# PolyChord/PolyChordLite

Hardware: AMD Instinct MI355X
Metric: likelihood evals/sec, 20D Gaussian nlive=2000 (higher is better)
Workload: dtype f64; 1 GPU; configs[1]: 20-D Gaussian, nlive=2000, num_repeats=40, one full run per step; batch_chains=1000, parallelism=repeat-sharded x1, mode=one run at a time per GPU; R runs in step: roofline.in_step

## Files before the change

### polychordlite_amd/csrc/pc_engine.hip

```cpp
#include "pc_state.h"
#include "pc_resume.h"
#include "pc_prior_table.h"
#include "pc_launch.h"
#include <cstdio>
#include <cstdlib>
#include <cstring>
#include <cstdarg>
#include <cmath>
#include <vector>
#include <memory>
#include <string>
#include <chrono>
#include <algorithm>
#include <map>
#include <unordered_map>
#include <atomic>
#include <mutex>
#include <thread>
#include <functional>
#include <exception>
#include <ucontext.h>
#include <array>
#include <sys/mman.h>
#include <unistd.h>
// ... 521 lines not shown
            case CK_CLUSG: { int nbm = 0, nmx = 0; for (size_t x = i; x < j; ++x) { nbm = std::max(nbm, ord[x]->ia[1]); nmx = std::max(nmx, ord[x]->ia[2]); } rc = pc_launch_knn_cluster_sub_many(d, cnt, nbm, nmx, q); } break;
            case CK_CLUS1: { int ndm = 0, nmx = 0, sub = 0; for (size_t x = i; x < j; ++x) { ndm = std::max(ndm, ord[x]->ia[1]); nmx = std::max(nmx, ord[x]->ia[2]); sub |= ord[x]->ia[3] > 0; } rc = pc_launch_knn_cluster_batch_many(&f.S, d, cnt, ndm, nmx, sub, q); } break;
            case CK_SORT: rc = pc_launch_sort_live_many(&f.S, d, cnt, q); break;
            case CK_CONSUME: rc = pc_launch_consume_par_many(&f.S, d, cnt, q); break;
            case CK_FINAL: rc = pc_launch_final_par_many(d, cnt, q); break;
            case CK_APPLY: rc = pc_launch_apply_many(&f.S, d, cnt, 0u, (int)f.a[0], q); break;
            case CK_UPDATE: { int nbm = 0; for (size_t x = i; x < j; ++x) nbm = std::max(nbm, ord[x]->ia[2]); rc = pc_launch_update_fused_many(&f.S, d, cnt, nbm, (int)f.a[0], (int)f.a[1], q); } break;
            }
            if (rc == 0) n_fused += cnt;
            else for (size_t x = i; x < j; ++x) { single(*ord[x], q); n_single++; }
            if (k == CK_BASES_NEXT && st2) {
                HIPCHK(hipEventRecord(ev_next, st2)); next_pending = true;
                if (!seq_open) { seq_launched++; seq_open = true; }
                if (!ev_seq[seq_launched & 3]) ev_seq[seq_launched & 3] = hpool().get_sync_event();
                HIPCHK(hipEventRecord(ev_seq[seq_launched & 3], st2));
            }
            i = j;
        }
        HIPCHK(hipEventRecord(ev[slot], st)); ev_used[slot] = true;
        if (used_st2 && ev2[slot]) { HIPCHK(hipEventRecord(ev2[slot], st2)); ev2_used[slot] = true; }
        pend.clear();
        seq_open = false;
        run_post();
    }
    void destroy()
    {
        for (int k = 0; k < 4; ++k) if (ev_seq[k]) { hpool().put_sync_event(ev_seq[k]); ev_seq[k] = nullptr; }
        for (int k = 0; k < RING; ++k) {
            if (ev_used[k]) (void)hipEventSynchronize(ev[k]);
            if (ev2_used[k]) (void)hipEventSynchronize(ev2[k]);
            if (ev[k]) hpool().put_sync_event(ev[k]);
            if (ev2[k]) hpool().put_sync_event(ev2[k]);
            ev2[k] = nullptr; ev2_used[k] = false;
            if (h_stage[k]) hfree(h_stage[k]);
            if (d_recs[k]) dfree(d_recs[k]);
            ev[k] = nullptr; h_stage[k] = nullptr; d_recs[k] = nullptr; ev_used[k] = false;
        }
        cap = 0;
    }
};

static std::atomic<long long> g_dbg_compact_ns{0}, g_dbg_nursery_ns{0}, g_dbg_capacity_ns{0}, g_dbg_endb_ns{0}, g_dbg_destroy_ns{0}, g_dbg_evwait_ns{0}, g_dbg_d1{0}, g_dbg_d2{0};
struct Engine {
    Cohort *co = nullptr;
    Fiber *fib = nullptr;
    pchip_settings cfg{};
    std::atomic<int> stop{0};
    polychord_batch_fn batch_fn = nullptr; void *batch_user = nullptr;
    polychord_loglike_fn cb_like = nullptr; polychord_prior_fn cb_prior = nullptr;
    bool callback_mode = false;
    void *d_cs = nullptr; double *d_x0s = nullptr, *d_prop = nullptr;
    int *d_decks = nullptr;
    double *hp_prop = nullptr, *hp_ans = nullptr, *d_ans = nullptr; int *hp_need = nullptr;
    long long cb_evals = 0; long cb_ticks = 0;
    std::vector<int> cb_idx; std::vector<double> cb_c, cb_t, cb_p, cb_l;
    polychord_dumper_fn dumper = nullptr;
    pchip_update_fn on_update = nullptr; void *hook_user = nullptr;
    long ndiscarded = 0;
    bool resume_static = true; unsigned resume_batch0 = 0;
    bool nph_stale = false;
    std::vector<double> hm_dead, hm_logw; int hm_ndead = 0;
    std::vector<unsigned> hm_cuid;
    std::vector<double> pp_rows, pp_logpost; std::vector<unsigned> pp_cuid; std::vector<unsigned long long> pp_uid; int nd_last_update = 0;
    std::vector<unsigned> split_child, split_parent; std::vector<double> split_logfrac;
    std::vector<double> h_lo, h_hi;
    PcState S{};
    hipStream_t st = nullptr;
    hipStream_t st_copy = nullptr;
    bool st_copy_shared = false;
    hipStream_t st_side = nullptr;
    hipEvent_t ev_main = nullptr;
    static constexpr int RAW_RING = 4;
    struct RawSlot { hipEvent_t ready = nullptr, consumed = nullptr; unsigned batch = 0; int B = 0; bool valid = false, waited = false, used = false; int co_seq = 0; };
    RawSlot ring[RAW_RING];
    int raw_depth = 2;
    double *h_dead = nullptr; size_t h_dead_cap = 0, h_dead_copied = 0;
    PcCtl *h_ctl = nullptr;
    PcCtl *h_note = nullptr;
    unsigned note_seq = 0;
    hipEvent_t ev_apply = nullptr;
    double *raw_buf[RAW_RING] = {nullptr, nullptr, nullptr, nullptr};
    double *ph2 = nullptr, *phL2 = nullptr; unsigned *phC2 = nullptr; unsigned long long *phU2 = nullptr;
    unsigned char *keep = nullptr; int *blk = nullptr, *d_total = nullptr;
    double *psum = nullptr, *mean = nullptr, *pcov = nullptr; int *pcnt = nullptr, *count = nullptr;
    size_t cov_chunks_cap = 0;
    double *upd_part = nullptr, *upd_shift = nullptr; size_t upd_part_cap = 0;
    PcPriorTable ptab; bool have_ptab = false;
    double *d_lo = nullptr, *d_hi = nullptr, *d_invcovT = nullptr, *d_mean = nullptr, *d_src = nullptr;
    double *d_dynL = nullptr; int *d_dynN = nullptr; double *d_logn = nullptr;
    double *c_Sm = nullptr; int *c_pts = nullptr, *c_gidx = nullptr, *c_knn = nullptr, *c_lab = nullptr, *c_out = nullptr, *c_cnt = nullptr;
    unsigned *c_olduid = nullptr; int c_cap = 0;
    long nsplits = 0; int ncluster_peak = 1;
    bool src_terms = false;
    long path[PCHIP_PATH_COUNT] = {};
    Timing tm;
    KTimer kt;
    int B = 0, dev = 0;
    bool fast_ok = false;
    bool cb_auto_batch = false; int B_small = 1; double cb_eval_seconds = -1.0;
    long long nlike_g[PC_MAX_GRADE] = {0};
    std::vector<int> h_nlike_g;

    void alloc_phantom_side(int Pcap)
    {
        ph2 = dalloc<double>((size_t)Pcap * S.nT); phL2 = dalloc<double>(Pcap); phC2 = dalloc<unsigned>(Pcap);
        phU2 = dalloc<unsigned long long>(Pcap); keep = dalloc<unsigned char>(Pcap); blk = dalloc<int>((Pcap + 255) / 256 + 1);
    }

    std::vector<void *> setup_staged;
    void upload(void *dst, const void *src, size_t bytes)
    {
        void *h = halloc<char>(bytes);
        setup_staged.push_back(h);
        std::memcpy(h, src, bytes);
        HIPCHK(hipMemcpyAsync(dst, h, bytes, hipMemcpyHostToDevice, st));
    }
    void setup(const pchip_settings &c, const pchip_like &like, const pchip_prior &prior)
    {
        cfg = c;
        { std::lock_guard<std::mutex> g(g_cb_mutex); batch_fn = g_batch_fn; batch_user = g_batch_user; }
        int ndev = 0;
        if (hipGetDeviceCount(&ndev) != hipSuccess || ndev == 0) {
            engine_fail(PC_RC_DEVICE, "no HIP device available -- this engine has no CPU path");
        }
        dev = c.device >= 0 ? c.device % ndev : 0;
        HIPCHK(hipSetDevice(dev));
        st = co ? co->st : hpool().get_stream();
        st_copy = (co && co->stc[0]) ? co->stc[(co->n_stc++) & 1] : (co ? hpool().get_stream() : stream_beside({st}));
        st_copy_shared = co && co->stc[0];
        kt.on = c.profile != 0 && !co; kt.st = st;
        kt.mask = (c.profile == 1) ? 0xFFFFFFFFu : (((unsigned)c.profile >> 1) & 0x7Fu);
        kt.stride = std::max(1u, ((unsigned)c.profile >> 8) & 0xFFu);
        const int D = c.nDims, nDer = c.nDerived;
        S.D = D; S.nDer = nDer; S.nT = 2 * D + nDer + 2; S.nr = c.num_repeats; S.N = c.nlive;
        S.ngrade = 1; S.g_off[0] = 0; S.g_nr[0] = c.num_repeats;
        for (int g = 1; g < PC_MAX_GRADE; ++g) { S.g_off[g] = 0; S.g_nr[g] = 0; }
        if (c.nGrade > 1 && c.grade_dims && c.grade_repeats) {
            if (c.nGrade > PC_MAX_GRADE) engine_fail(PC_RC_SETTINGS, "at most %d parameter grades", PC_MAX_GRADE);
            S.ngrade = c.nGrade;
            int off = 0, tot = 0;
            for (int g = 0; g < c.nGrade; ++g) {
                if (c.grade_dims[g] < 1 || c.grade_repeats[g] < 1) engine_fail(PC_RC_SETTINGS, "every grade needs at least one parameter and one repeat");
                S.g_off[g] = off; off += c.grade_dims[g]; S.g_nr[g] = c.grade_repeats[g]; tot += c.grade_repeats[g];
            }
            if (off != D) engine_fail(PC_RC_SETTINGS, "grade_dims must sum to nDims");
            S.nr = tot; cfg.num_repeats = tot;
        }
        S.nb_total = 0; S.n_dev = 0;
        for (int g = 0, col = 0; g < PC_MAX_GRADE; ++g) {
            const int Dg = D - S.g_off[g];
            S.g_nb[g] = g < S.ngrade ? (S.g_nr[g] + Dg - 1) / Dg : 0;
            S.g_col0[g] = col; S.g_e0[g] = (int)S.n_dev;
            col += S.g_nr[g]; S.nb_total += S.g_nb[g]; S.n_dev += (unsigned)S.g_nb[g] * Dg * Dg;
        }
        sub_dims.clear();
        if (c.n_sub_cluster < 0 || (c.n_sub_cluster > 0 && !c.sub_cluster_dims)) engine_fail(PC_RC_SETTINGS, "n_sub_cluster = %d without a list of coordinates", c.n_sub_cluster);
        for (int k = 0; k < c.n_sub_cluster; ++k) {
            const int d = c.sub_cluster_dims[k];
            if (d < 0 || d >= D) engine_fail(PC_RC_SETTINGS, "sub-clustering coordinate %d out of range (nDims = %d; the indices are 0-based)", d, D);
            if (std::find(sub_dims.begin(), sub_dims.end(), d) != sub_dims.end()) engine_fail(PC_RC_SETTINGS, "sub-clustering coordinate %d given twice", d);
            sub_dims.push_back(d);
        }
        S.ch_nlike_g = nullptr;
        std::memset(nlike_g, 0, sizeof(nlike_g));
        S.p0 = D; S.d0 = 2 * D; S.b0 = 2 * D + nDer; S.l0 = S.b0 + 1;
        int nmax = c.nlive;
        for (int i = 0; i < c.n_nlives; ++i) nmax = std::max(nmax, c.nlives[i]);
        const int nprior = c.nprior <= 0 ? c.nlive : c.nprior;
        S.Ncap = std::max(nmax, nprior);
        B = c.batch > 0 ? c.batch : std::max(1, std::min(1024, c.nlive / 2));
        if (B > 65535) engine_fail(PC_RC_LIMIT, "batch = %d chains per nursery: at most 65535", B);
        if (c.sequential_rng) B = 1;
        cb_auto_batch = c.batch <= 0 && !c.sequential_rng && (like.kind == PC_LIKE_CALLBACK || (prior.kind != 1 && prior.kind != PCHIP_PRIOR_TABLE));
        if (cb_auto_batch) B_small = std::max(1, std::min(64, c.nlive / 4));
        S.B = B;
        S.maxc = c.do_clustering ? std::max(2, g_cap_clusters.load()) : 4;
        S.maxc_dead = 4096;
        S.Pcap = (int)std::min<long long>(2000000000LL / S.nT, 4LL * S.nr * S.Ncap + 4LL * B * S.nr + 1024);
        if (g_cap_phantoms.load() > 0) S.Pcap = std::max(g_cap_phantoms.load(), B * S.nr + 16);
        S.Dcap = 64 * S.Ncap + 4 * B + 1024;
        S.k0 = (uint32_t)c.seed; S.k1 = 0x504F4C59u;
        S.logzero = c.logzero; S.use_prec = c.precision_criterion > 0;
        S.log_prec = S.use_prec ? std::log(c.precision_criterion) : 0.0;
        S.log_cf = std::log(c.compression_factor);
        S.max_ndead = c.max_ndead; S.nfail = c.nfail <= 0 ? c.nlive : c.nfail;
        S.seed_override = 0; S.ablate = c.ablate; S.seq_mode = c.sequential_rng ? 1 : 0;
        S.epoch_discard = c.epoch_discard ? 1 : 0;
        if (S.seq_mode) { cfg.batch = 1; cfg.force_general = 1; }
        S.n_nlives = c.n_nlives;
        if (c.n_nlives > 0) {
            d_dynL = dalloc<double>(c.n_nlives); d_dynN = dalloc<int>(c.n_nlives);
            upload(d_dynL, c.loglikes, sizeof(double) * c.n_nlives);
            upload(d_dynN, c.nlives, sizeof(int) * c.n_nlives);
        }
        S.dyn_loglikes = d_dynL; S.dyn_nlives = d_dynN;
        S.like.kind = like.kind; S.like.mu = like.mu; S.like.sigma = like.sigma; S.like.logdetcov = like.logdetcov;
        S.like.norm = -(double)D * (std::log(like.sigma > 0 ? like.sigma : 1.0) + PC_LOG_TWO_PI / 2.0);
        S.like.inv_sigma = like.sigma > 0 ? 1.0 / like.sigma : 1.0;
        S.like.log_vn = 0.5 * D * std::log(3.14159265358979323846) - std::lgamma(1.0 + D / 2.0);
        S.like.invcov = nullptr; S.like.mean = nullptr;
        S.src_id = 0; S.src_pad = 0; S.src_data = nullptr; S.src_ndata = 0;
        if (like.kind == PC_LIKE_SOURCE) {
            const double *h = nullptr; long long n = 0;
            if (pc_rtc_source_data(like.source, &h, &n)) engine_fail(PC_RC_SETTINGS, "device source handle %d does not exist", like.source);
            if (nDer > PC_SRC_MAX_DERIVED) engine_fail(PC_RC_SETTINGS, "a device source likelihood writes at most %d derived parameters, not %d", PC_SRC_MAX_DERIVED, nDer);
            if (prior.kind != 1 && prior.kind != PCHIP_PRIOR_TABLE) engine_fail(PC_RC_SETTINGS, "a device source likelihood needs a device prior (the uniform box), not a host-callback prior");
            S.src_id = like.source;
            src_terms = pc_rtc_source_terms(like.source) > 0;
            if (n > 0) { d_src = dalloc<double>((size_t)n); upload(d_src, h, sizeof(double) * (size_t)n); S.src_data = d_src; S.src_ndata = n; }
        }
        if (like.kind == PC_LIKE_CORR_GAUSSIAN) {
            std::vector<double> T((size_t)D * D);
            for (int a = 0; a < D; ++a) for (int b = 0; b < D; ++b) T[(size_t)b * D + a] = like.invcov[(size_t)a * D + b];
            d_invcovT = dalloc<double>((size_t)D * D); d_mean = dalloc<double>(D);
            upload(d_invcovT, T.data(), sizeof(double) * D * D);
            upload(d_mean, like.mean, sizeof(double) * D);
            S.like.invcov = d_invcovT; S.like.mean = d_mean;
        }
        have_ptab = false;
        int prior_kind = prior.kind;
        std::vector<double> box_lo, box_hi;
        const double *p_lo = prior.lo, *p_hi = prior.hi;
        if (prior.kind == PCHIP_PRIOR_TABLE) {
            const std::string err = pc_prior_table_build(D, prior.table, prior.hyper, ptab);
            if (!err.empty()) { pc_abi_set_last_error(err.c_str()); engine_fail(PC_RC_SETTINGS, "%s", err.c_str()); }
            have_ptab = true;
            if (ptab.is_box && like.kind != PC_LIKE_CALLBACK) {
                box_lo.resize(D); box_hi.resize(D);
                for (int i = 0; i < D; ++i) { box_lo[i] = ptab.e[i].par[0]; box_hi[i] = ptab.e[i].par[1]; }
                prior_kind = 1; p_lo = box_lo.data(); p_hi = box_hi.data();
            }
        } else if (prior.kind != 0 && prior.kind != 1) engine_fail(PC_RC_SETTINGS, "prior.kind = %d: 0 (callback), 1 (uniform box) or 2 (table)", prior.kind);
        callback_mode = (like.kind == PC_LIKE_CALLBACK) || (prior_kind != 1 && prior_kind != PCHIP_PRIOR_TABLE);
        if (callback_mode) {
            cb_like = like.fn; cb_prior = prior.kind == PCHIP_PRIOR_TABLE ? nullptr : prior.fn;
            if (!cb_like) engine_fail(PC_RC_SETTINGS, "callback mode needs a loglikelihood function pointer");
        }
        S.prior.kind = callback_mode ? (prior_kind == PCHIP_PRIOR_TABLE ? 0 : prior_kind) : prior_kind; S.prior.lo = nullptr; S.prior.hi = nullptr;
        if (prior_kind == 1 && p_lo && p_hi) {
            d_lo = dalloc<double>(D); d_hi = dalloc<double>(D);
            upload(d_lo, p_lo, sizeof(double) * D);
            upload(d_hi, p_hi, sizeof(double) * D);
            S.prior.lo = d_lo; S.prior.hi = d_hi;
        }
        if (S.prior.kind == PCHIP_PRIOR_TABLE) {
            const std::vector<double> tp = ptab.dev_par(); const std::vector<int> ti = ptab.dev_int();
            d_lo = dalloc<double>(tp.size()); d_hi = dalloc<double>((ti.size() + 1) / 2);
            upload(d_lo, tp.data(), sizeof(double) * tp.size());
            upload(d_hi, ti.data(), sizeof(int) * ti.size());
            S.prior.lo = d_lo; S.prior.hi = d_hi; S.src_pad = (int)ptab.mask;
        }
        const int Ncap = S.Ncap, maxc = S.maxc, nT = S.nT, nr = S.nr;
        S.live = dalloc<double>((size_t)Ncap * nT); S.live_logL = dalloc<double>(Ncap);
        S.live_cluster = dalloc<int>(Ncap); S.live_pos = dalloc<int>(Ncap); S.live_entry = dalloc<double>(Ncap);
        S.cl_list = dalloc<int>((size_t)maxc * Ncap); S.cl_n = dalloc<int>(maxc);
        S.logZp = dalloc<double>(maxc); S.logXp = dalloc<double>(maxc); S.logZXp = dalloc<double>(maxc);
        S.logZp2 = dalloc<double>(maxc); S.logZpXp = dalloc<double>(maxc); S.logLp = dalloc<double>(maxc);
        S.XpXq = dalloc<double>(2 * (size_t)maxc * maxc); S.imin_slot = dalloc<int>(maxc);
        S.lse_ref = dalloc<double>(maxc); S.lse_sum = dalloc<double>(maxc); S.death_thr = dalloc<double>(maxc);
        S.cl_uid = dalloc<unsigned>(maxc);
        S.chol = dalloc<double>((size_t)maxc * D * D); S.cov = dalloc<double>((size_t)maxc * D * D);
        S.logZp_dead = dalloc<double>(S.maxc_dead); S.logZp2_dead = dalloc<double>(S.maxc_dead); S.cl_uid_dead = dalloc<unsigned>(S.maxc_dead);
        S.phantom = dalloc<double>((size_t)S.Pcap * nT); S.ph_logL = dalloc<double>(S.Pcap);
        S.ph_cuid = dalloc<unsigned>(S.Pcap); S.ph_uid = dalloc<unsigned long long>(S.Pcap);
        alloc_phantom_side(S.Pcap);
        S.dead = dalloc<double>((size_t)S.Dcap * nT); S.dead_logw = dalloc<double>(S.Dcap);
        S.dead_postX = dalloc<double>(S.Dcap); S.dead_postZ = dalloc<double>(S.Dcap); S.dead_cuid = dalloc<unsigned>(S.Dcap);
        S.dead_entry = dalloc<double>(S.Dcap);
        S.babies = dalloc<double>((size_t)B * nr * nT); S.baby_logL = dalloc<double>((size_t)B * nr); S.baby_logL_T = dalloc<double>((size_t)B * nr);
        S.ch_cluster = dalloc<int>(B); S.ch_epoch = dalloc<int>(B); S.ch_nlike = dalloc<int>(B); S.ch_seed_slot = dalloc<int>(B);
        S.ch_contour = dalloc<double>(B);
        if (S.ngrade > 1) { S.ch_nlike_g = dalloc<int>((size_t)B * PC_MAX_GRADE); h_nlike_g.assign((size_t)B * PC_MAX_GRADE, 0); }
        {
            std::vector<double> ln((size_t)Ncap + 4);
            ln[0] = -PC_HUGE;
            for (int k = 1; k < Ncap + 4; ++k) ln[k] = std::log((double)k);
            d_logn = dalloc<double>(ln.size());
            upload(d_logn, ln.data(), sizeof(double) * ln.size());
            S.logn = d_logn;
        }
        S.nn_list = nullptr; S.nn_slot_owner = nullptr; S.nn_chain_slot = nullptr; S.nn_pts = nullptr; S.nn_code = nullptr; S.nn_valid = 0;
        if (c.do_clustering) {
            S.nn_list = dalloc<int>((size_t)B * nr * PC_NN_K); S.nn_slot_owner = dalloc<int>(Ncap); S.nn_chain_slot = dalloc<int>(B);
            S.nn_pts = dalloc<double>((size_t)(Ncap + B) * D); S.nn_code = dalloc<int>((size_t)2 * Ncap + B + 64);
            if (!sub_dims.empty()) { c_subdims = dalloc<int>(sub_dims.size()); upload(c_subdims, sub_dims.data(), sizeof(int) * sub_dims.size()); }
        }
        S.nhat = dalloc<double>((size_t)B * nr * D); S.nhat_w = dalloc<double>((size_t)B * nr);
        static const bool ms_off = std::getenv("PC_MS_PRE_OFF") != nullptr;
        const bool ms_pre = S.like.kind == PC_LIKE_CORR_GAUSSIAN && D > 64 && D <= 128 && S.ngrade <= 1 && !S.seq_mode && !(S.ablate & 1) && !ms_off && S.prior.kind != PCHIP_PRIOR_TABLE;
        S.nhat_Ms = ms_pre ? dalloc<double>((size_t)B * nr * D) : nullptr;
        S.ch_My = ms_pre ? dalloc<double>((size_t)B * D) : nullptr;
        static const bool split_off = std::getenv("PC_NHATS_SPLIT_OFF") != nullptr;
        const bool split_q = D > 64 && D <= 128 && S.ngrade <= 1 && !S.seq_mode && !split_off && !callback_mode;
        const bool split_m = D > 24 && D <= 64 && S.ngrade <= 1 && !S.seq_mode && !split_off && !callback_mode;
        const size_t raw_n = split_q ? (size_t)B * S.nb_total * 32 * 512 : split_m ? (size_t)B * S.nb_total * (D <= 32 ? 1024 : 4096) : (size_t)B * S.nb_total * D * D + (size_t)B * 33 + 8;
        S.nhat_raw = ((D <= 24 && !S.seq_mode && !split_off) || split_q || split_m) ? dalloc<double>(raw_n)
                   : (D > 128 ? dalloc<double>((size_t)B * S.nb_total * D * 256) : nullptr);
        static const int depth_env = std::getenv("PC_RAW_DEPTH") ? std::max(2, std::min(RAW_RING, std::atoi(std::getenv("PC_RAW_DEPTH")))) : 3;
        raw_depth = split_q ? RAW_RING : depth_env;
        raw_buf[0] = S.nhat_raw;
        for (int r = 1; r < raw_depth; ++r) raw_buf[r] = ((D <= 24 || split_q || split_m) && S.nhat_raw) ? dalloc<double>(raw_n) : nullptr;
        S.plan = dalloc<PcPlan>(B); S.slot_src = dalloc<int>(Ncap); S.slot_step = dalloc<int>(Ncap); S.slot_dead = dalloc<int>(Ncap); HIPCHK(hipMemsetAsync(S.slot_dead, 0xFF, sizeof(int) * Ncap, st)); S.defer_update = 0; S.sort_slot = dalloc<int>(Ncap + 64); S.sort_key = dalloc<unsigned long long>(Ncap + 64);
        S.ctl = dalloc<PcCtl>(1);
        d_total = dalloc<int>(1);
        if (callback_mode) {
            d_cs = (void *)dalloc<char>(pc_chain_state_size() * B); d_x0s = dalloc<double>((size_t)B * D); d_prop = dalloc<double>((size_t)B * D);
            const size_t nans = (size_t)B * (1 + D + std::max(1, nDer));
            d_ans = dalloc<double>(nans);
            d_decks = dalloc<int>((size_t)B * nr);
            hp_prop = halloc<double>((size_t)B * D); hp_ans = halloc<double>(nans); hp_need = halloc<int>(B);
            std::memset(hp_ans, 0, sizeof(double) * nans); std::memset(hp_need, 0, sizeof(int) * B);
            HIPCHK(hipMemset(d_cs, 0, pc_chain_state_size() * B));
        }
        h_ctl = halloc<PcCtl>(1);
        h_note = halloc<PcCtl>(1);
        std::memset(h_note, 0, sizeof(PcCtl)); note_seq = 0;
        { void *dp = nullptr; HIPCHK(hipHostGetDevicePointer(&dp, h_note, 0)); S.ctl_host = (PcCtl *)dp; }
        S.notify_seq = 0;
        pc_launch_init_state(&S, c.logzero, st);
        PcCtl c0{};
        c0.status = PC_ST_RUNNING; c0.ncluster = 1; c0.logZ = c.logzero; c0.logZ2 = c.logzero;
        c0.logX_last_update = 0.0; c0.next_cluster_uid = 1; c0.live_logZ = c.logzero;
        *h_ctl = c0;
    }

    void grade_counts(long *o)
    {
        for (int g = 0; g < PC_MAX_GRADE; ++g) o[g] = 0;
        if (S.ngrade <= 1) { o[0] = (long)h_ctl->nlike; return; }
        long rest = 0;
        for (int g = 1; g < S.ngrade; ++g) { o[g] = (long)nlike_g[g]; rest += o[g]; }
        o[0] = (long)h_ctl->nlike - rest;
    }

    void tally_grades()
    {
        if (S.ngrade <= 1) return;
        for (int w = h_ctl->seg_lo; w <= h_ctl->seg_hi; ++w)
            for (int g = 0; g < PC_MAX_GRADE; ++g) nlike_g[g] += h_nlike_g[(size_t)w * PC_MAX_GRADE + g];
    }

    void sync_point()
    {
        if (fib) {
            fib->yield();
            if (fib->cancel) {
                for (const Fetch &f : fetching) hfree(f.h);
                fetching.clear(); own_fetches.clear();
                for (void *h : staged_up) hfree(h);
                staged_up.clear();
                throw FiberCancelled{};
            }
            return;
        }
        if (co) co->flush();
        for (int spins = 0; spins < 200000; ++spins) { const hipError_t q = hipStreamQuery(st); if (q != hipErrorNotReady) { HIPCHK(q); break; } __builtin_ia32_pause(); }
        HIPCHK(hipStreamSynchronize(st));
    }
    void direct_op() { if (co) co->flush(); }
    struct Fetch { void *h; void *dst; size_t bytes; };
    std::vector<Fetch> fetching;
    void fetch_raw(void *dst, const void *src, size_t bytes)
    {
        if (!bytes) return;
        void *h = halloc<char>(bytes);
        fetching.push_back({h, dst, bytes});
        hipStream_t q = st;
        if (co && batch_copies()) co->post_copies.push_back({(uintptr_t)h, (uintptr_t)src, (uintptr_t)bytes});
        else if (co) co->post.push_back([h, src, bytes, q] { HIPCHK(hipMemcpyAsync(h, src, bytes, hipMemcpyDeviceToHost, q)); });
        else if (batch_copies()) own_fetches.push_back({(uintptr_t)h, (uintptr_t)src, (uintptr_t)bytes});
        else HIPCHK(hipMemcpyAsync(h, src, bytes, hipMemcpyDeviceToHost, st));
    }
    template <class T> void fetch(std::vector<T> &v, const T *p, size_t n) { v.resize(n); fetch_raw(v.data(), p, sizeof(T) * n); }
    std::vector<std::array<uintptr_t, 3>> own_fetches;
    void fetch_wait()
    {
        if (!own_fetches.empty()) { std::vector<std::array<uintptr_t, 3>> c; c.swap(own_fetches); pc_copy_many(c, st); }
        sync_point();
        for (const Fetch &f : fetching) { std::memcpy(f.dst, f.h, f.bytes); hfree(f.h); }
        fetching.clear();
        for (void *h : staged_up) hfree(h);
        staged_up.clear();
    }
    std::vector<void *> staged_up;
    void send_raw(void *dst, const void *src, size_t bytes)
    {
        if (!bytes) return;
        direct_op();
        void *h = halloc<char>(bytes);
        staged_up.push_back(h);
        std::memcpy(h, src, bytes);
        if (co && batch_copies()) co->pre_copies.push_back({(uintptr_t)dst, (uintptr_t)h, (uintptr_t)bytes});
        else HIPCHK(hipMemcpyAsync(dst, h, bytes, hipMemcpyHostToDevice, st));
    }

    void send_pre(void *dst, const void *src, size_t bytes)
    {
        if (!bytes) return;
        if (!co) { send_raw(dst, src, bytes); return; }
        void *h = halloc<char>(bytes);
        staged_up.push_back(h);
        std::memcpy(h, src, bytes);
        hipStream_t q = st;
        if (batch_copies()) co->pre_copies.push_back({(uintptr_t)dst, (uintptr_t)h, (uintptr_t)bytes});
        else co->pre.push_back([dst, h, bytes, q] { HIPCHK(hipMemcpyAsync(dst, h, bytes, hipMemcpyHostToDevice, q)); });
    }
    static bool batch_copies() { static const bool off = std::getenv("PC_COPY_BATCH_OFF") != nullptr; return !off; }

    void read_ctl()
    {
        fetch_raw(h_ctl_in(), S.ctl, sizeof(PcCtl));
        fetch_wait();
        *h_ctl = ctl_in;
        HIPCHK(hipGetLastError());
        nph_stale = false;
        kt.collect();
    }
    PcCtl ctl_in;
    PcCtl *h_ctl_in() { return &ctl_in; }

    void launch_stamp() { S.notify_seq = ++note_seq; }
    unsigned long ready_spins = 0;
    bool round_ready()
    {
        static const bool off = std::getenv("PC_NOTIFY_OFF") != nullptr;
        if (off || !S.ctl_host) { read_ctl(); return true; }
        const volatile unsigned long long *w = (const volatile unsigned long long *)h_note;
        unsigned long long got[PC_NOTE_WORDS];
        bool all = true;
        for (int i = 0; i < PC_NOTE_WORDS; ++i) { got[i] = w[i]; all = all && (unsigned)(got[i] >> 32) == note_seq; }
        if (!all) {
            if ((++ready_spins & 0x3FFFu) == 0x3FFFu) {
                const hipError_t q = hipStreamQuery(st);
                if (q == hipSuccess) {
                    bool ok = true;
                    for (int i = 0; i < PC_NOTE_WORDS; ++i) ok = ok && (unsigned)(w[i] >> 32) == note_seq;
                    if (!ok) engine_fail(PC_RC_DEVICE, "a contraction kernel finished without reporting (launch failure?)");
                } else if (q != hipErrorNotReady) engine_fail(PC_RC_DEVICE, "HIP error %s while waiting for a round", hipGetErrorString(q));
                if (ready_spins > (1ul << 22)) std::this_thread::yield();
            }
            return false;
        }
        PcCtl &c = *h_ctl;
        const int hi_before = c.i_nursery > 0 ? c.i_nursery - 1 : B - 1;
        c.status = (int)(got[0] & 0xFF); c.error = (int)((got[0] >> 8) & 0xFF); c.cluster_deleted = (int)((got[0] >> 16) & 1);
        c.upd_pending = (int)((got[0] >> 17) & 1); c.upd_marks = (int)((got[0] >> 18) & 0x3FFF);
        c.i_nursery = (int)((unsigned)got[1] & 0xFFFFu); c.ndead = (int)(unsigned)got[2]; c.nphantom = (int)(unsigned)got[3];
        c.ncluster = (int)(got[4] & 0xFFFF);
        {
            int cand = (c.ncluster_dead & ~0xFFFF) | (int)((got[4] >> 16) & 0xFFFF);
            if (cand < c.ncluster_dead) cand += 0x10000;
            c.ncluster_dead = cand;
        }
        c.seg_hi = hi_before; c.seg_lo = c.i_nursery;
        nph_stale = false;
        return true;
    }

    void grow_dead(int nd)
    {
        if (co) co->flush();
        HIPCHK(hipStreamSynchronize(st_copy));
        auto grow = [&](auto *&p, size_t per) {
            using T = std::remove_reference_t<decltype(*p)>;
            T *q = dalloc<T>((size_t)nd * per);
            HIPCHK(hipMemcpyAsync(q, p, sizeof(T) * (size_t)h_ctl->ndead * per, hipMemcpyDeviceToDevice, st));
            HIPCHK(hipStreamSynchronize(st));
            dfree(p); p = q;
        };
        grow(S.dead, S.nT); grow(S.dead_logw, 1); grow(S.dead_postX, 1); grow(S.dead_postZ, 1); grow(S.dead_cuid, 1); grow(S.dead_entry, 1);
        S.Dcap = nd;
        if (h_dead && (size_t)nd > h_dead_cap) { hfree(h_dead); h_dead_cap = (size_t)nd; h_dead = halloc<double>(h_dead_cap * S.nT); h_dead_copied = 0; }
    }

    void grow_phantoms(long long need)
    {
        if (co) co->flush();
        const long long hard = 1LL << 30;
        if (need > hard) engine_fail(PC_RC_LIMIT, "more than %lld phantom points (%lld needed)", hard, need);
        long long np = std::max<long long>(need, 2LL * S.Pcap);
        np = std::min(np, hard);
        if (g_inject_fault.load() == 3) { g_inject_fault = 0; engine_fail(PC_RC_MEMORY, "out of device memory growing the phantom array to %lld rows (injected)", np); }
        const size_t used = (size_t)std::min<long long>(h_ctl->nphantom, S.Pcap);
        HIPCHK(hipStreamSynchronize(st));
        auto grow = [&](auto *&p, size_t per) {
            using T = std::remove_reference_t<decltype(*p)>;
            T *q = dalloc<T>((size_t)np * per);
            if (used) HIPCHK(hipMemcpyAsync(q, p, sizeof(T) * used * per, hipMemcpyDeviceToDevice, st));
            HIPCHK(hipStreamSynchronize(st));
            dfree(p); p = q;
        };
        grow(S.phantom, S.nT); grow(S.ph_logL, 1); grow(S.ph_cuid, 1); grow(S.ph_uid, 1);
        dfree(ph2); dfree(phL2); dfree(phC2); dfree(phU2); dfree(keep); dfree(blk);
        alloc_phantom_side((int)np);
        S.Pcap = (int)np;
    }

    long long pool_cursor = 0;
    double *babies_own = nullptr;
    bool compact_wanted() const { return S.pool && h_ctl->status == PC_ST_RUNNING && h_ctl->i_nursery == 0 && pool_cursor + (long long)B * S.nr > S.Pcap; }
    void compact_record() { co->rec(CK_COMPACT, S, {keep, blk, d_total, ph2, phL2, phC2, phU2}, {}, {0, (int)pool_cursor, ((int)pool_cursor + 255) / 256}); }
    void compact_finish(int total)
    {
        std::swap(S.phantom, ph2); std::swap(S.ph_logL, phL2); std::swap(S.ph_cuid, phC2); std::swap(S.ph_uid, phU2);
        pool_cursor = total; h_ctl->nphantom = total; nph_stale = false;
        if (pool_cursor + (long long)B * S.nr > S.Pcap / 2) grow_phantoms(std::max<long long>(2LL * S.Pcap, 2 * (pool_cursor + (long long)B * S.nr)));
        tm.compactions++;
    }
    void pool_compact()
    {
        const auto dbg_t0 = std::chrono::steady_clock::now();
        struct DbgT { std::chrono::steady_clock::time_point t0; ~DbgT() { g_dbg_compact_ns += std::chrono::duration_cast<std::chrono::nanoseconds>(std::chrono::steady_clock::now() - t0).count(); } } dbg_t{dbg_t0};
        if (co) co->flush();
        hipEvent_t e0 = kt.begin(KT_CLEAN);
        pc_launch_clean(&S, (int)pool_cursor, keep, blk, d_total, ph2, phL2, phC2, phU2, nullptr, st);
        kt.end(KT_CLEAN, e0);
        int total = 0;
        HIPCHK(hipMemcpyAsync(&total, d_total, sizeof(int), hipMemcpyDeviceToHost, st));
        HIPCHK(hipStreamSynchronize(st));
        kt.collect();
        compact_finish(total);
    }
    void ensure_capacity()
    {
        if ((long long)h_ctl->ndead + B + S.Ncap + 16 > S.Dcap) grow_dead(S.Dcap * 2);
        if (S.pool) { if (h_ctl->ncluster_dead + h_ctl->ncluster + 8 > S.maxc_dead) grow_dead_clusters(2 * S.maxc_dead); return; }
        if (nph_stale && (long long)h_ctl->nphantom + (long long)B * S.nr > S.Pcap) read_ctl();
        if ((long long)h_ctl->nphantom + (long long)B * S.nr > S.Pcap) grow_phantoms((long long)h_ctl->nphantom + (long long)B * S.nr);
        if (h_ctl->ncluster_dead + h_ctl->ncluster + 8 > S.maxc_dead) grow_dead_clusters(2 * S.maxc_dead);
    }

    void grow_dead_clusters(int nd)
    {
        if (co) co->flush();
        HIPCHK(hipStreamSynchronize(st));
        const size_t used = (size_t)std::min(h_ctl->ncluster_dead, S.maxc_dead);
        auto grow = [&](auto *&p) {
            using T = std::remove_reference_t<decltype(*p)>;
            T *q = dalloc<T>((size_t)nd);
            if (used) HIPCHK(hipMemcpy(q, p, sizeof(T) * used, hipMemcpyDeviceToDevice));
            dfree(p); p = q;
        };
        grow(S.logZp_dead); grow(S.logZp2_dead); grow(S.cl_uid_dead);
        S.maxc_dead = nd;
    }

    void grow_clusters(int need)
    {
        const int mo = S.maxc, mn = std::max(need, 2 * mo), Ncap = S.Ncap, DD = S.D * S.D;
        if (mn > 16384) engine_fail(PC_RC_LIMIT, "more than 16384 clusters");
        if (co) co->flush();
        HIPCHK(hipStreamSynchronize(st));
        auto grow_d = [&](double *&p, double fill) {
            std::vector<double> v = dl(p, (size_t)mo); v.resize(mn, fill);
            dfree(p); p = dalloc<double>(mn); ul(p, v);
        };
        grow_d(S.logZp, cfg.logzero); grow_d(S.logZXp, cfg.logzero); grow_d(S.logZp2, cfg.logzero); grow_d(S.logZpXp, cfg.logzero);
        grow_d(S.logLp, cfg.logzero); grow_d(S.logXp, 0.0); grow_d(S.lse_ref, 0.0); grow_d(S.lse_sum, 0.0); grow_d(S.death_thr, -PC_HUGE);
        { std::vector<int> v = dl(S.cl_n, (size_t)mo); v.resize(mn, 0); dfree(S.cl_n); S.cl_n = dalloc<int>(mn); ul(S.cl_n, v); }
        { std::vector<int> v = dl(S.imin_slot, (size_t)mo); v.resize(mn, 0); dfree(S.imin_slot); S.imin_slot = dalloc<int>(mn); ul(S.imin_slot, v); }
        { std::vector<unsigned> v = dl(S.cl_uid, (size_t)mo); v.resize(mn, 0u); dfree(S.cl_uid); S.cl_uid = dalloc<unsigned>(mn); ul(S.cl_uid, v); }
        {
            std::vector<double> o = dl(S.XpXq, (size_t)mo * mo), v((size_t)mn * mn, 0.0);
            for (int a = 0; a < mo; ++a) std::copy(o.begin() + (size_t)a * mo, o.begin() + (size_t)(a + 1) * mo, v.begin() + (size_t)a * mn);
            dfree(S.XpXq); S.XpXq = dalloc<double>(2 * (size_t)mn * mn); ul(S.XpXq, v);
        }
        {
            int *q = dalloc<int>((size_t)mn * Ncap);
            HIPCHK(hipMemcpy(q, S.cl_list, sizeof(int) * (size_t)mo * Ncap, hipMemcpyDeviceToDevice));
            dfree(S.cl_list); S.cl_list = q;
        }
        auto grow_mat = [&](double *&p) {
            double *q = dalloc<double>((size_t)mn * DD);
            HIPCHK(hipMemcpy(q, p, sizeof(double) * (size_t)mo * DD, hipMemcpyDeviceToDevice));
            std::vector<double> id((size_t)(mn - mo) * DD, 0.0);
            for (int c = 0; c < mn - mo; ++c) for (int a = 0; a < S.D; ++a) id[(size_t)c * DD + (size_t)a * S.D + a] = 1.0;
            HIPCHK(hipMemcpy(q + (size_t)mo * DD, id.data(), sizeof(double) * id.size(), hipMemcpyHostToDevice));
            dfree(p); p = q;
        };
        grow_mat(S.chol); grow_mat(S.cov);
        if (c_cnt) { dfree(c_cnt); dfree(c_olduid); c_cnt = dalloc<int>(mn); c_olduid = dalloc<unsigned>(mn); }
        dfree(psum); dfree(pcnt); dfree(pcov); dfree(mean); dfree(count); cov_chunks_cap = 0;
        S.maxc = mn;
    }

    void call_dumper(int stage = 0)
    {
        if (!(dumper && stage != 2) && !on_update) return;
        const int nT = S.nT, D = S.D, nDer = S.nDer, npars = D + nDer + 2, nd = h_ctl->ndead;
        HIPCHK(hipStreamSynchronize(st));
        if (nd > hm_ndead) {
            std::vector<double> rows((size_t)(nd - hm_ndead) * nT), lw(nd - hm_ndead);
            hm_cuid.resize(nd);
            HIPCHK(hipMemcpy(hm_cuid.data() + hm_ndead, S.dead_cuid + hm_ndead, sizeof(unsigned) * (nd - hm_ndead), hipMemcpyDeviceToHost));
            HIPCHK(hipMemcpy(rows.data(), S.dead + (size_t)hm_ndead * nT, sizeof(double) * rows.size(), hipMemcpyDeviceToHost));
            HIPCHK(hipMemcpy(lw.data(), S.dead_logw + hm_ndead, sizeof(double) * lw.size(), hipMemcpyDeviceToHost));
            hm_dead.resize((size_t)nd * npars); hm_logw.resize(nd);
            for (int i = hm_ndead; i < nd; ++i) {
                const double *r = rows.data() + (size_t)(i - hm_ndead) * nT;
                double *o = hm_dead.data() + (size_t)i * npars;
                std::memcpy(o, r + S.p0, sizeof(double) * (D + nDer)); o[D + nDer] = r[S.b0]; o[D + nDer + 1] = r[S.l0];
                hm_logw[i] = lw[i - hm_ndead] + r[S.l0];
            }
            hm_ndead = nd;
        }
        std::vector<double> lwn(hm_logw.begin(), hm_logw.begin() + nd);
        double m = -PC_HUGE;
// ... 1781 lines not shown
```

### polychordlite_amd/csrc/pc_launch.h

```cpp
#pragma once
#include "pc_state.h"
#include "../../include/polychord_hip.h"
#include <cstddef>

static inline int pc_slice_phi_lds(const PcState *S)
{
    const size_t sh0 = sizeof(double) * ((size_t)S->D + S->nr) + 16, tb = sizeof(double) * (size_t)S->nr * (S->D + 1);
    return (S->nDer > 0 && sh0 + tb <= 48 * 1024) ? 1 : 0;
}

extern "C" {

void pc_abi_set_last_error(const char *msg);
void pc_launch_slice_tick(const PcState *S, unsigned batch, int nchains, void *cs, double *x0s, int *decks, double *prop, const double *ev_logL,
                          const double *ev_theta, const double *ev_phi, int first, double *prop_host, int *need_host, hipStream_t st);
size_t pc_chain_state_size(void);
int pc_launch_killoff_cl(const PcState *S, int nc, hipStream_t st);
int pc_consume_cl_fits(const PcState *S, int nc);
int pc_consume_clp_fits(const PcState *S, int nc);
int pc_launch_consume_cl_many(const PcState *S, const PcManyRec *dR, int R, int wide, hipStream_t st);
int pc_launch_consume_cl(const PcState *S, int nc, hipStream_t st);
int pc_launch_knn_cluster_sub(const int *d_desc, int nb, int mmax, const double *Sm, const int *pool, int *knn, int *labels, int *out, hipStream_t st);
int pc_launch_knn_cluster_sub_many(const PcManyRec *dR, int R, int nb_max, int mmax, hipStream_t st);
void pc_launch_remap_chains(const PcState *S, const int *map, int nold, int n, hipStream_t st);
void pc_launch_shift_mats(const PcState *S, int p, int nc, hipStream_t st);
void pc_launch_similarity(const PcState *S, const int *pts, int n, double *Sm, const int *dims, int nd, hipStream_t st);
int pc_launch_knn_cluster(const double *Sm, int nroot, const int *gidx, int m, int *knn, int *labels, int *out, hipStream_t st);
int pc_launch_knn_cluster_batch(const PcState *S, const int *h_desc, const int *d_desc, int nd, double *Sm, int *knn, int *labels, int *out, const int *dims, int ndims, hipStream_t st);
int pc_launch_knn_cluster_batch_dev(const PcState *S, const int *d_desc, int nd, int nmax, double *Sm, int *knn, int *labels, int *out, const int *dims, int ndims, hipStream_t st);
int pc_launch_knn_cluster_batch_many(const PcState *S, const PcManyRec *dR, int R, int nd_max, int nmax, int any_sub, hipStream_t st);
void pc_launch_rebuild(const PcState *S, int nc, hipStream_t st);
void pc_launch_ph_rehome(const PcState *S, int nph, int nc, const unsigned *old_uids, int nold_uids, int *counts, hipStream_t st);
void pc_launch_nn_lists(const PcState *S, int nleft, int use_rank, hipStream_t st);
int pc_launch_nn_lists_many(const PcState *S, const PcManyRec *dR, int R, int nleft_max, int use_rank, hipStream_t st);
int pc_launch_consume(const PcState *S, int final_mode, int wide, hipStream_t st);
void pc_launch_apply(const PcState *S, unsigned batch, int nchains, hipStream_t st);
int pc_launch_apply_many(const PcState *S, const PcManyRec *dR, int R, unsigned batch, int nchains, hipStream_t st);
int pc_launch_clean_many(const PcManyRec *dR, int R, int nblk_max, hipStream_t st);
void pc_launch_install_live(const PcState *S, const double *rows, int n, hipStream_t st);
void pc_launch_clean(const PcState *S, int nph, unsigned char *keep, int *blk, int *d_total, double *ph2, double *phL2, unsigned *phC2, unsigned long long *phU2, int *dst_index, hipStream_t st);
void pc_launch_reset_thresholds(const PcState *S, hipStream_t st);
int pc_launch_reset_thresholds_many(const PcState *S, const PcManyRec *dR, int R, hipStream_t st);
int pc_cov_nchunk(const PcState *S, int nph);
int pc_launch_covmats(const PcState *S, int nph, int nc, double *psum, int *pcnt, double *mean, int *count, double *pcov, hipStream_t st);
void pc_launch_scan_blocks(int *blk, int nblk, int *total, int *total2, hipStream_t st);
void pc_launch_chol_only(const PcState *S, const double *ncov, const int *count, hipStream_t st);
void pc_launch_init_state(const PcState *S, double logzero, hipStream_t st);
int pc_post_blocks(void);
void pc_launch_post_moments(const PcState *S, int nd, double *pmax, double *part, hipStream_t st);
void pc_prepare_streams(int dev, int want);
void *pc_cache_dev_alloc(size_t bytes);
void pc_cache_dev_free(void *p);
void *pc_cache_host_alloc(size_t bytes);
void pc_cache_host_free(void *p);
int pc_run_many(const pchip_settings *s, const pchip_like *like, const pchip_prior *prior, int nseeds, const int *seeds, int device, int max_in_flight, pchip_result *results);
int pc_fast_fits(const PcState *S);
int pc_launch_sort_live(const PcState *S, hipStream_t st);
int pc_launch_sort_live_many(const PcState *S, const PcManyRec *dR, int R, hipStream_t st);
int pc_launch_consume_fast(const PcState *S, int final_mode, hipStream_t st);
void pc_launch_ph_prepare(const PcState *S, hipStream_t st);
size_t pc_records_block_bytes(long long cap, int nT);
int pc_pack_lived_device(const double *dead, const double *logw, const double *entry, long long nd, int nT, double logzero, double *block, long long cap, long long *h_count, hipStream_t st);
int pc_par_fits(const PcState *S);
int pc_launch_consume_par(const PcState *S, hipStream_t st);
int pc_launch_consume_par_many(const PcState *S, const PcManyRec *dR, int R, hipStream_t st);
int pc_launch_final_par(const PcState *S, hipStream_t st);
int pc_launch_final_par_many(const PcManyRec *dR, int R, hipStream_t st);
int pc_rtc_launch(const PcState *S, const char *expr, dim3 grid, dim3 block, size_t sh, hipStream_t st, void **args);
const char *pc_rtc_error(void);
int pc_rtc_source_data(int id, const double **data, long long *n);
long pc_rtc_source_terms(int id);
int pc_rtc_wanted(const PcState *S);
int pc_launch_generate_live(const PcState *S, int attempt0, int n, double *rows, double *rows_logL, hipStream_t st);
int pc_nhats_splittable(const PcState *S);
int pc_launch_nhats_part(const PcState *S, unsigned batch, int nchains, int part, hipStream_t st, int packed);
int pc_launch_nhats(const PcState *S, unsigned batch, int nchains, hipStream_t st);
int pc_slice_fusable(const PcState *S);
int pc_launch_slice_fused(const PcState *S, unsigned batch, int nchains, hipStream_t st);
int pc_launch_slice_many(const PcState *S, const PcManyRec *dR, int R, int nchains, int fused, hipStream_t st);
int pc_launch_nhats_many(const PcState *S, const PcManyRec *dR, int R, int nchains, hipStream_t st);
int pc_launch_slice(const PcState *S, unsigned batch, int nchains, hipStream_t st);
int pc_launch_prior_transform(const PcState *S, int n, const double *cubes, double *thetas, hipStream_t st);
int pc_launch_source_eval(const PcState *S, int n, const double *thetas, double *logL, double *phi, hipStream_t st);
int pc_bases_t_ok(const PcState *S);
int pc_launch_bases_t(const PcState *S, unsigned batch, int nchains, hipStream_t st);
int pc_launch_bases_t_many(const PcState *S, const PcManyRec *dR, int R, unsigned batch, int nchains, hipStream_t st);
int pc_slice_t_ok(const PcState *S, int ncluster);
int pc_launch_slice_t(const PcState *S, unsigned batch, int nchains, hipStream_t st);
int pc_launch_slice_t_many(const PcState *S, const PcManyRec *dR, int R, unsigned batch, int nchains, hipStream_t st);
int pc_update_fused_ok(const PcState *S, int nc);
int pc_update_fused_blocks(const PcState *S, int nph);
int pc_update_fused_entries(const PcState *S);
void pc_launch_update_fused(const PcState *S, int nph, unsigned char *keep, int *blk, int *d_total, double *ph2, double *phL2, unsigned *phC2,
                            unsigned long long *phU2, double *part, double *shift, int deferred, hipStream_t st);
int pc_update_fused_grid(const PcState *S, int nph, int deferred);
int pc_launch_update_fused_many(const PcState *S, const PcManyRec *dR, int R, int nblk_max, int G, int deferred, hipStream_t st);

}
```

### polychordlite_amd/csrc/pc_update.hip

```cpp
#include "pc_state.h"
#include "pc_launch.h"
#include <atomic>
#include <cstdio>
#include <cstdlib>

#define UPD_ROWS 256
#define UPD_NT 256

__device__ __forceinline__ void upd_stage_masked(const double *src0, unsigned long long mask, unsigned long long mmask, double *dst,
                                                 double *tile, int TS, const double *sh, int D, int nT, int lane)
{
    const int ne = dst ? nT : D + 1;
    int n = 0;
    while (mask) {
        int idx[16], cnt = 0;
#pragma unroll
        for (int u = 0; u < 16; ++u) {
            idx[u] = 0;
            if (mask) { idx[u] = __ffsll((long long)mask) - 1; mask &= mask - 1; cnt = u + 1; }
        }
        for (int e = lane; e < ne; e += 64) {
            double v[16];
#pragma unroll
            for (int u = 0; u < 16; ++u) if (u < cnt) v[u] = (e < nT) ? src0[(size_t)idx[u] * nT + e] : 0.0;
            if (dst) {
#pragma unroll
                for (int u = 0; u < 16; ++u) if (u < cnt) dst[(size_t)(n + u) * nT + e] = v[u];
            }
            if (e <= D) {
                const double s = e < D ? sh[e] : 0.0;
#pragma unroll
                for (int u = 0; u < 16; ++u)
                    if (u < cnt && ((mmask >> idx[u]) & 1ull))
                        tile[(size_t)__popcll(mmask & ((1ull << idx[u]) - 1ull)) * TS + e] = e < D ? v[u] - s : 1.0;
            }
        }
        n += cnt;
    }
}

__device__ __forceinline__ void upd_flag_body(const PcState &S, int nph, unsigned char *keep, int *blk_count, int def, int nblk)
{
    const int tid = threadIdx.x, lane = tid & 63, wv = tid >> 6;
    const int sb = blockIdx.x * 4 + wv;
    if (sb >= nblk) return;
    const unsigned uid0 = S.cl_uid[0];
    const double thr = def ? S.ctl->upd_thr : S.death_thr[0];
    const bool pool = S.pool;
    const int tmark = (pool && def) ? S.ctl->upd_tmark : 0x7fffffff, nph0u = (pool && def) ? S.ctl->upd_nph0 : 0x7fffffff;
    const int T = (pool && def) ? S.ctl->upd_T : 0, nr = S.nr;
    const int j0 = sb * UPD_ROWS + 4 * lane;
    const bool full = j0 + 3 < nph;
    unsigned cu[4] = {PC_CUID_NONE, PC_CUID_NONE, PC_CUID_NONE, PC_CUID_NONE};
    double ll[4] = {0.0, 0.0, 0.0, 0.0};
    if (full) {
        const uint4 c = *(const uint4 *)(S.ph_cuid + j0);
        const double2 a = *(const double2 *)(S.ph_logL + j0), b2 = *(const double2 *)(S.ph_logL + j0 + 2);
        cu[0] = c.x; cu[1] = c.y; cu[2] = c.z; cu[3] = c.w; ll[0] = a.x; ll[1] = a.y; ll[2] = b2.x; ll[3] = b2.y;
    } else {
        for (int u = 0; u < 4; ++u) if (j0 + u < nph) { cu[u] = S.ph_cuid[j0 + u]; ll[u] = S.ph_logL[j0 + u]; }
    }
    unsigned kb = 0; bool wr = false; int cnt = 0;
#pragma unroll
    for (int u = 0; u < 4; ++u) {
        const int j = j0 + u;
        bool k = false, km = false;
        if (j < nph) {
            k = (cu[u] == uid0) && !(ll[u] < thr);
            if (pool) {
                if (!k && cu[u] == uid0) { cu[u] = PC_CUID_NONE; wr = true; }
                km = k && (j < nph0u || T - 1 - (j - nph0u) / nr < tmark);
            }
            kb |= (unsigned)((k ? 1 : 0) | (km ? 2 : 0)) << (8 * u);
        }
        cnt += __popcll(__ballot(pool ? km : k));
    }
    if (full) {
        *(unsigned *)(keep + j0) = kb;
        if (wr) *(uint4 *)(S.ph_cuid + j0) = make_uint4(cu[0], cu[1], cu[2], cu[3]);
    } else {
        for (int u = 0; u < 4; ++u) if (j0 + u < nph) { keep[j0 + u] = (unsigned char)((kb >> (8 * u)) & 0xFFu); if (wr) S.ph_cuid[j0 + u] = cu[u]; }
    }
    if (lane == 0) blk_count[sb] = cnt;
}
__global__ __launch_bounds__(UPD_NT) void k_upd_flag(PcState S, int nph, unsigned char *keep, int *blk_count, int def, int nblk) { upd_flag_body(S, nph, keep, blk_count, def, nblk); }
__global__ __launch_bounds__(UPD_NT) void k_upd_flag_many(const PcManyRec *R, int def) { const PcManyView r = pc_many_view(R, blockIdx.y); if ((int)blockIdx.x * 4 >= r.ia[2]) return; upd_flag_body(r.S, r.ia[1], (unsigned char *)r.p[0], (int *)r.p[1], def, r.ia[2]); }


__global__ __launch_bounds__(1024) void k_upd_scan(int *cnt, int n, int *total)
{
    __shared__ int wsum[16];
    __shared__ int carry_s;
    const int tid = threadIdx.x, lane = tid & 63, wv = tid >> 6;
    int carry = 0;
    for (int base = 0; base < n; base += 4096) {
        const int i0 = base + 4 * tid;
        int c[4];
#pragma unroll
        for (int u = 0; u < 4; ++u) c[u] = (i0 + u < n) ? cnt[i0 + u] : 0;
        const int s = (c[0] + c[1]) + (c[2] + c[3]);
        int inc = s;
#pragma unroll
        for (int o = 1; o < 64; o <<= 1) { const int t = __shfl_up(inc, o); if (lane >= o) inc += t; }
        if (lane == 63) wsum[wv] = inc;
        __syncthreads();
        int pre = carry;
        for (int x = 0; x < wv; ++x) pre += wsum[x];
        int run = pre + inc - s;
#pragma unroll
        for (int u = 0; u < 4; ++u) { if (i0 + u < n) cnt[i0 + u] = run; run += c[u]; }
        if (tid == 1023) carry_s = pre + inc;
        __syncthreads();
        carry = carry_s;
    }
    if (tid == 0) *total = carry;
}

__global__ __launch_bounds__(UPD_NT) void k_upd_index(int nph, const unsigned char *keep, const int *blk_off, int *idx)
{
    __shared__ int cnt[4];
    const int tid = threadIdx.x, lane = tid & 63, wv = tid >> 6;
    const int j = blockIdx.x * UPD_ROWS + tid;
    const bool km = j < nph && (keep[j] & 2);
    const unsigned long long m = __ballot(km);
    if (lane == 0) cnt[wv] = __popcll(m);
    __syncthreads();
    int off = blk_off[blockIdx.x];
    for (int x = 0; x < wv; ++x) off += cnt[x];
    if (km) idx[off + __popcll(m & ((1ull << lane) - 1ull))] = j;
}

#define UPD_SELF_BLOCKS 4096
#define UPD_IDX_NT 256
#define UPD_IDX_BLOCKS 16
__device__ __forceinline__ void upd_index_self_body(int nph, const unsigned char *keep, const int *blk_count, int nblk, int *idx, int *total)
{
    __shared__ int part[4];
    const int tid = threadIdx.x, lane = tid & 63, wv = tid >> 6;
    const int sb0 = blockIdx.x * UPD_IDX_BLOCKS;
    int s = 0;
    for (int b = tid; b < sb0; b += UPD_IDX_NT) s += blk_count[b];
#pragma unroll
    for (int o = 32; o >= 1; o >>= 1) s += __shfl_xor(s, o);
    if (lane == 0) part[wv] = s;
    __syncthreads();
    int off = (part[0] + part[1]) + (part[2] + part[3]);
    const int sbw = sb0 + 4 * wv;
    for (int x = sb0; x < sbw && x < nblk; ++x) off += blk_count[x];
    const unsigned long long below = (1ull << lane) - 1ull;
    for (int q = 0; q < 4; ++q) {
        const int sb = sbw + q;
        if (sb >= nblk) return;
        const int j0 = sb * UPD_ROWS + 4 * lane;
        unsigned w = 0;
        if (j0 + 3 < nph) w = *(const unsigned *)(keep + j0);
        else for (int u = 0; u < 4; ++u) if (j0 + u < nph) w |= (unsigned)keep[j0 + u] << (8 * u);
        int pos = off, all = 0;
        bool f[4];
#pragma unroll
        for (int u = 0; u < 4; ++u) {
            f[u] = (w >> (8 * u + 1)) & 1u;
            const unsigned long long m = __ballot(f[u]);
            pos += __popcll(m & below); all += __popcll(m);
        }
#pragma unroll
        for (int u = 0; u < 4; ++u) if (f[u]) { idx[pos] = j0 + u; pos++; }
        off += all;
        if (sb == nblk - 1 && lane == 0) *total = off;
    }
}
__global__ __launch_bounds__(UPD_IDX_NT) void k_upd_index_self(int nph, const unsigned char *keep, const int *blk_count, int nblk, int *idx, int *total) { upd_index_self_body(nph, keep, blk_count, nblk, idx, total); }
__global__ __launch_bounds__(UPD_IDX_NT) void k_upd_index_self_many(const PcManyRec *R) { const PcManyView r = pc_many_view(R, blockIdx.y); if ((int)blockIdx.x * 16 >= r.ia[2]) return; upd_index_self_body(r.ia[1], (const unsigned char *)r.p[0], (const int *)r.p[1], r.ia[2], (int *)r.p[5], (int *)r.p[2]); }


__device__ __forceinline__ void upd_stage_idx(const double *base, const int *ridx, int cnt, double *tile, int TS, const double *sh, int D, int nT, int lane)
{
    if (cnt <= 0) return;
    int idx[16];
#pragma unroll
    for (int u = 0; u < 16; ++u) idx[u] = u < cnt ? ridx[u] : 0;
    for (int e0 = lane; e0 <= D; e0 += 128) {
        const int e1 = e0 + 64;
        double v0[16], v1[16];
#pragma unroll
        for (int u = 0; u < 16; ++u) if (u < cnt) { v0[u] = e0 < D ? base[(size_t)idx[u] * nT + e0] : 1.0; v1[u] = e1 < D ? base[(size_t)idx[u] * nT + e1] : 1.0; }
        const double s0 = e0 < D ? sh[e0] : 0.0, s1 = e1 < D ? sh[e1] : 0.0;
#pragma unroll
        for (int u = 0; u < 16; ++u) if (u < cnt) { tile[(size_t)u * TS + e0] = v0[u] - s0; if (e1 <= D) tile[(size_t)u * TS + e1] = v1[u] - s1; }
    }
}

typedef double upd_v4d __attribute__((ext_vector_type(4)));
template <int NT, int W>
__device__ __forceinline__ void updg_accumulate(const double *tile, int TS, int n16, int wv, int li, int lk, upd_v4d (&acc)[(NT <= 2) ? NT * (NT + 1) / 2 : (NT * (NT + 1) / 2 + 3) / 4])
{
    if constexpr (NT <= 2) {
        for (int q0 = 4 * wv; q0 < n16; q0 += 16) {
            const double *row = tile + (size_t)(q0 + lk) * TS + li;
            double x[NT];
#pragma unroll
            for (int t = 0; t < NT; ++t) x[t] = row[16 * t];
            int q = 0;
#pragma unroll
            for (int ti = 0; ti < NT; ++ti)
#pragma unroll
                for (int tj = ti; tj < NT; ++tj, ++q) acc[q] = __builtin_amdgcn_mfma_f64_16x16x4f64(x[ti], x[tj], acc[q], 0, 0, 0);
        }
    } else {
        for (int ks = 0; ks < (n16 >> 2); ++ks) {
            const double *row = tile + (size_t)(4 * ks + lk) * TS + li;
            double x[NT];
#pragma unroll
            for (int t = 0; t < NT; ++t) x[t] = row[16 * t];
            int q = 0;
#pragma unroll
            for (int ti = 0; ti < NT; ++ti)
#pragma unroll
                for (int tj = ti; tj < NT; ++tj, ++q)
                    if ((q & 3) == W) acc[q >> 2] = __builtin_amdgcn_mfma_f64_16x16x4f64(x[ti], x[tj], acc[q >> 2], 0, 0, 0);
        }
    }
}
__device__ __forceinline__ int updg_slot(int D, int ti, int tj, int li, int lk, int r)
{
    const int a = 16 * ti + lk + 4 * r, b = 16 * tj + li, npair = D * (D + 1) / 2;
    if (a > b || b > D) return -1;
    return (b < D) ? a * D - a * (a - 1) / 2 + (b - a) : (a < D ? npair + a : npair + D);
}

template <int NT, bool IDX>
__device__ __forceinline__ void upd_gather_body(const PcState &S, int nph, int nblk, const unsigned char *keep, const int *blk_off,
                                                double *ph2, double *phL2, unsigned *phC2, unsigned long long *phU2,
                                                const int *idx, const int *nidx_p,
                                                const double *shift, double *part, int E, int def, int nlb, int ndb)
{
    extern __shared__ __attribute__((aligned(16))) char smem[];
    constexpr bool KS = NT <= 2;
    constexpr int TS = KS ? 16 * NT + 1 : 16 * NT + ((NT & 1) ? 0 : 16);
    constexpr int CAP = KS ? 128 : 64;
    constexpr int NACC = KS ? NT * (NT + 1) / 2 : (NT * (NT + 1) / 2 + 3) / 4;
    __shared__ unsigned long long m64[4], mm64[4];
    __shared__ long long dix[256];
    const int tmark = def ? S.ctl->upd_tmark : 0x7fffffff, nph0u = def ? S.ctl->upd_nph0 : 0x7fffffff, updT = def ? S.ctl->upd_T : 0;
    const int tid = threadIdx.x, lane = tid & 63, wv = tid >> 6, li = lane & 15, lk = lane >> 4, D = S.D, nT = S.nT;
    constexpr bool pool = IDX;
    double *tile = (double *)smem;
    double *sh = tile + (size_t)CAP * TS;
    for (int d = tid; d < D; d += 256) sh[d] = shift[d];
    for (int e = tid; e < CAP * TS; e += 256) tile[e] = 0.0;
    upd_v4d acc[NACC];
#pragma unroll
    for (int t = 0; t < NACC; ++t) acc[t] = upd_v4d{0.0, 0.0, 0.0, 0.0};
    int nfill = 0;
    auto flush = [&]() __attribute__((always_inline)) {
        __syncthreads();
        const int n16 = (nfill + 15) & ~15;
        for (int e = tid; e < (n16 - nfill) * (D + 1); e += 256) tile[(size_t)(nfill + e / (D + 1)) * TS + e % (D + 1)] = 0.0;
        __syncthreads();
        if (KS || wv == 0) updg_accumulate<NT, 0>(tile, TS, n16, wv, li, lk, acc);
        else if (wv == 1) updg_accumulate<NT, 1>(tile, TS, n16, wv, li, lk, acc);
        else if (wv == 2) updg_accumulate<NT, 2>(tile, TS, n16, wv, li, lk, acc);
        else updg_accumulate<NT, 3>(tile, TS, n16, wv, li, lk, acc);
        __syncthreads();
        nfill = 0;
    };
    auto piece = [&](const double *src, int sub, double *dst) __attribute__((always_inline)) {
        const unsigned long long ms = m64[sub], mms = mm64[sub], below = (1ull << (16 * wv)) - 1ull;
        const int cnt = __popcll(mms);
        if (cnt == 0 && (dst == nullptr || ms == 0ull)) return;
        if (nfill + cnt > CAP) flush();
        upd_stage_masked(src + (size_t)(sub * 64 + 16 * wv) * nT, ((dst ? ms : mms) >> (16 * wv)) & 0xFFFFull, (mms >> (16 * wv)) & 0xFFFFull,
                         dst ? dst + (size_t)__popcll(ms & below) * nT : nullptr, tile + (size_t)(nfill + __popcll(mms & below)) * TS, TS, sh, D, nT, lane);
        nfill += cnt;
    };
    if constexpr (IDX) {
        const int nidx = *nidx_p;
        const int gchunk = (int)gridDim.x - nlb - ndb;
        for (int c = blockIdx.x; (int)blockIdx.x < gchunk && c * 64 < nidx; c += gchunk) {
            const int have = min(64, nidx - c * 64);
            if (nfill + have > CAP) flush();
            upd_stage_idx(S.phantom, idx + c * 64 + 16 * wv, min(16, have - 16 * wv), tile + (size_t)(nfill + 16 * wv) * TS, TS, sh, D, nT, lane);
            nfill += have;
        }
    }
    const int total = nblk + nlb + ndb;
    for (int b = IDX ? ((int)blockIdx.x >= (int)gridDim.x - nlb - ndb ? nblk + (int)blockIdx.x - ((int)gridDim.x - nlb - ndb) : total) : blockIdx.x; b < total; b += gridDim.x) {
        __syncthreads();
        if (b < nblk) {
            const int j = b * 256 + tid;
            const bool k = (j < nph) && keep[j];
            const bool km = k && (j < nph0u || (pool ? updT - 1 - (j - nph0u) / S.nr : (j - nph0u) / S.nr) < tmark);
            const unsigned long long m = __ballot(k), mm = __ballot(km);
            if (lane == 0) { m64[wv] = m; mm64[wv] = mm; }
            __syncthreads();
            int off = 0;
            if (!pool) {
                off = blk_off[b];
                for (int x = 0; x < wv; ++x) off += __popcll(m64[x]);
                if (k) {
                    const int pos = off + __popcll(m & ((1ull << lane) - 1ull));
                    phL2[pos] = S.ph_logL[j]; phC2[pos] = S.ph_cuid[j]; phU2[pos] = S.ph_uid[j];
                }
                off = blk_off[b];
            }
            const double *src = S.phantom + (size_t)b * 256 * nT;
            for (int sub = 0; sub < 4; ++sub) {
                piece(src, sub, pool ? nullptr : ph2 + (size_t)off * nT);
                off += __popcll(m64[sub]);
            }
        } else if (b < nblk + nlb) {
            const int r0 = (b - nblk) * 256, r = r0 + tid;
            const bool k = (r < S.Ncap) && S.live_cluster[r] == 0 && (!def || S.slot_step[r] < tmark);
            const unsigned long long m = __ballot(k);
            if (lane == 0) { m64[wv] = m; mm64[wv] = m; }
            __syncthreads();
            const double *src = S.live + (size_t)r0 * nT;
            for (int sub = 0; sub < 4; ++sub) piece(src, sub, nullptr);
        } else {
            const PcCtl *ctl = S.ctl;
            const int T = ctl->upd_T, ts = ctl->upd_ts;
            const int t = tmark + (b - nblk - nlb) * 256 + tid;
            long long di = -1;
            if (t < ts) {
                const PcPlan *pw = S.plan + (T - 1 - t);
                const int src = pw->dead_src;
                const bool existed = src >= 0 || (T - 1 - (-src - 1)) < tmark;
                if (pw->dead_idx >= 0 && pw->logw > S.logzero && existed) di = pw->dead_idx;
            }
            dix[tid] = di;
            const unsigned long long m = __ballot(di >= 0);
            if (lane == 0) m64[wv] = m;
            __syncthreads();
            for (int sub = 0; sub < 4; ++sub) {
                unsigned long long mb = m64[sub];
                const int cnt = __popcll(mb);
                if (cnt == 0) continue;
                if (nfill + cnt > CAP) flush();
                int row = 0;
                while (mb) {
                    const int bit = __ffsll((long long)mb) - 1; mb &= mb - 1;
                    if ((row & 3) == wv) {
                        const long long d = dix[sub * 64 + bit];
                        for (int e = lane; e <= D; e += 64) tile[(size_t)(nfill + row) * TS + e] = e < D ? S.dead[(size_t)d * nT + e] - sh[e] : 1.0;
                    }
                    row++;
                }
                nfill += cnt;
            }
        }
    }
    flush();
    double *out = part + (size_t)blockIdx.x * E;
    if constexpr (KS) {
        double *wres = tile;
#pragma unroll
        for (int t = 0; t < NACC; ++t)
#pragma unroll
            for (int r = 0; r < 4; ++r) wres[((size_t)wv * NACC + t) * 256 + (lk + 4 * r) * 16 + li] = acc[t][r];
        __syncthreads();
        if (wv == 0) {
            int q = 0;
#pragma unroll
            for (int ti = 0; ti < NT; ++ti)
#pragma unroll
                for (int tj = ti; tj < NT; ++tj, ++q)
#pragma unroll
                    for (int r = 0; r < 4; ++r) {
                        const int p = updg_slot(D, ti, tj, li, lk, r), idx = (lk + 4 * r) * 16 + li;
                        if (p >= 0) out[p] = ((wres[(size_t)(0 * NACC + q) * 256 + idx] + wres[(size_t)(1 * NACC + q) * 256 + idx]) +
                                              (wres[(size_t)(2 * NACC + q) * 256 + idx] + wres[(size_t)(3 * NACC + q) * 256 + idx]));
                    }
        }
    } else {
        int q = 0;
#pragma unroll
        for (int ti = 0; ti < NT; ++ti)
#pragma unroll
            for (int tj = ti; tj < NT; ++tj, ++q)
                if ((q & 3) == wv) {
#pragma unroll
                    for (int r = 0; r < 4; ++r) { const int p = updg_slot(D, ti, tj, li, lk, r); if (p >= 0) out[p] = acc[q >> 2][r]; }
                }
    }
}
template <int NT, bool IDX>
__global__ __launch_bounds__(256) void k_upd_gather(PcState S, int nph, int nblk, const unsigned char *keep, const int *blk_off,
                                                    double *ph2, double *phL2, unsigned *phC2, unsigned long long *phU2,
                                                    const int *idx, const int *nidx_p,
                                                    const double *shift, double *part, int E, int def, int nlb, int ndb)
{ upd_gather_body<NT, IDX>(S, nph, nblk, keep, blk_off, ph2, phL2, phC2, phU2, idx, nidx_p, shift, part, E, def, nlb, ndb); }
template <int NT>
__global__ __launch_bounds__(256) void k_upd_gather_many(const PcManyRec *R, int E, int def, int nlb, int ndb)
{
    const PcManyView r = pc_many_view(R, blockIdx.y);
    upd_gather_body<NT, true>(r.S, r.ia[1], r.ia[2], (const unsigned char *)r.p[0], (const int *)r.p[1], (double *)r.p[3], (double *)r.p[4], (unsigned *)r.p[5],
                              (unsigned long long *)r.p[6], (const int *)r.p[5], (const int *)r.p[2], (const double *)r.p[8], (double *)r.p[7], E, def, nlb, ndb);
}


#define UPD_FOLD 16
__device__ __forceinline__ void upd_fold_body(const double *part, int nb, int E, double *part2)
{
    const int g = blockIdx.x;
    for (int e = threadIdx.x; e < E; e += 256) {
        double t[UPD_FOLD];
#pragma unroll
        for (int u = 0; u < UPD_FOLD; ++u) t[u] = (g * UPD_FOLD + u < nb) ? part[(size_t)(g * UPD_FOLD + u) * E + e] : 0.0;
        double s = 0.0;
#pragma unroll
        for (int u = 0; u < UPD_FOLD; ++u) s += t[u];
        part2[(size_t)g * E + e] = s;
    }
}
__global__ __launch_bounds__(256) void k_upd_fold(const double *part, int nb, int E, double *part2) { upd_fold_body(part, nb, E, part2); }
__global__ __launch_bounds__(256) void k_upd_fold_many(const PcManyRec *R, int nb, int E) { double *part = pc_as_global((double *)R[blockIdx.y].p[7], R); upd_fold_body(part, nb, E, part + (size_t)nb * E); }


__device__ __forceinline__ void upd_final_body(const PcState &S, int nb, const double *part, int E, double *shift, int def)
{
    __shared__ double acc[4][256];
    __shared__ double A[32 * 32], L[32 * 32], mu[32];
    __shared__ int bad;
    const int tid = threadIdx.x, D = S.D, npair = D * (D + 1) / 2, nE = npair + D + 1;
    __shared__ double tot[544];
    for (int e0 = 0; e0 < nE; e0 += 256) {
        const int e = e0 + (tid & 255), h = tid >> 8;
        double s = 0.0;
        if (e < nE) {
            for (int k = h; k < nb; k += 4 * 16) {
                double t[16];
#pragma unroll
                for (int u = 0; u < 16; ++u) t[u] = (k + 4 * u < nb) ? part[(size_t)(k + 4 * u) * E + e] : 0.0;
#pragma unroll
                for (int u = 0; u < 16; ++u) s += t[u];
            }
        }
        acc[h][tid & 255] = s;
        __syncthreads();
        if (tid < 256 && e < nE) tot[e] = (acc[0][tid] + acc[1][tid]) + (acc[2][tid] + acc[3][tid]);
        __syncthreads();
    }
#ifdef UPD_DBG
    const long long f0 = clock64();
#endif
    if (tid == 0) bad = 0;
    const double n = tot[npair + D];
    if (tid < D) mu[tid] = tot[npair + tid] / n;
    __syncthreads();
    for (int p = tid; p < D * D; p += 1024) {
        const int a = p / D, b = p % D, lo = a < b ? a : b, hi = a < b ? b : a;
        const int idx = lo * D - lo * (lo - 1) / 2 + (hi - lo);
        const double c = tot[idx] / n - mu[lo] * mu[hi];
        A[p] = c; L[p] = 0.0;
        S.cov[p] = c;
    }
    __syncthreads();
#ifdef UPD_DBG
    const long long f1 = clock64();
#endif
    if (tid < 64) {
        double a[32];
#pragma unroll
        for (int k = 0; k < 32; ++k) a[k] = (tid < D && k < D) ? A[tid * D + k] : 0.0;
        bool fail = false;
#pragma unroll
        for (int i = 0; i < 32; ++i) {
            if (i < D && !fail) {
                const double aii = readlane_f64(a[i], i);
                if (aii <= 0.0) fail = true;
                else {
                    const double lii = sqrt(aii);
                    const double lji = (tid == i) ? lii : a[i] / lii;
                    if (tid >= i) a[i] = lji;
#pragma unroll
                    for (int k = i + 1; k < 32; ++k)
                        if (k < D) { const double lki = readlane_f64(lji, k); if (tid > i) a[k] -= lji * lki; }
                }
            }
        }
        if (fail) { if (tid == 0) bad = 1; }
        else if (tid < D) {
#pragma unroll
            for (int k = 0; k < 32; ++k) if (k < D) L[tid * D + k] = (k <= tid) ? a[k] : 0.0;
        }
    }
    __syncthreads();
    if (bad) {
        double tr = 0.0;
        for (int k = 0; k < D; ++k) tr += A[k * D + k];
        for (int p = tid; p < D * D; p += 1024) L[p] = (p / D == p % D) ? sqrt(tr) : 0.0;
        __syncthreads();
    }
    for (int p = tid; p < D * D; p += 1024) S.chol[p] = L[p];
    if (tid < D) shift[tid] += mu[tid];
    if (tid == 0) { if (!(def && S.ctl->upd_keep_thr)) S.death_thr[0] = -PC_HUGE; if (def) S.ctl->upd_pending = 0; }
#ifdef UPD_DBG
    if (tid == 0) { const long long f2 = clock64(); S.ctl->gen_cyc[2] += f1 - f0; S.ctl->gen_cyc[3] += f2 - f1; S.ctl->nn_walks += f0; }
#endif
}
__global__ __launch_bounds__(1024) void k_upd_final(PcState S, int nb, const double *part, int E, double *shift, int def) { upd_final_body(S, nb, part, E, shift, def); }
__global__ __launch_bounds__(1024) void k_upd_final_many(const PcManyRec *R, int nb, int E, int def, int G) { const PcManyView r = pc_many_view(R, blockIdx.y); upd_final_body(r.S, nb, (const double *)r.p[7] + (size_t)G * E, E, (double *)r.p[8], def); }


__global__ __launch_bounds__(1024) void k_upd_final_w(PcState S, int nb, const double *part, int E, double *shift, int def, double *ncov, int *count)
{
    extern __shared__ __attribute__((aligned(16))) char smem[];
    double *tot = (double *)smem;
    __shared__ double mu[128];
    const int tid = threadIdx.x, D = S.D, npair = D * (D + 1) / 2, nE = npair + D + 1;
    for (int e = tid; e < nE; e += 1024) {
        double s = 0.0;
        for (int k = 0; k < nb; k += 8) {
            double t[8];
#pragma unroll
            for (int u = 0; u < 8; ++u) t[u] = (k + u < nb) ? part[(size_t)(k + u) * E + e] : 0.0;
#pragma unroll
            for (int u = 0; u < 8; ++u) s += t[u];
        }
        tot[e] = s;
    }
    __syncthreads();
    const double n = tot[npair + D];
    if (tid < D) mu[tid] = tot[npair + tid] / n;
    __syncthreads();
    for (int p = tid; p < D * D; p += 1024) {
        const int a = p / D, b = p % D, lo = a < b ? a : b, hi = a < b ? b : a;
        ncov[p] = tot[lo * D - lo * (lo - 1) / 2 + (hi - lo)] - n * mu[lo] * mu[hi];
    }
    if (tid < D) shift[tid] += mu[tid];
    if (tid == 0) { count[0] = (int)n; if (!(def && S.ctl->upd_keep_thr)) S.death_thr[0] = -PC_HUGE; if (def) S.ctl->upd_pending = 0; }
}

static int upd_grid(const PcState *S, int nph, int deferred)
{
    const int nblk = (nph + UPD_ROWS - 1) / UPD_ROWS, nlb = (S->Ncap + UPD_ROWS - 1) / UPD_ROWS, ndb = deferred ? (S->B + UPD_ROWS - 1) / UPD_ROWS : 0;
    static const int cap_env = std::getenv("PC_UPD_GRID") ? std::atoi(std::getenv("PC_UPD_GRID")) : 0;
    const int cap = cap_env > 0 ? cap_env : (S->D < 32 ? 384 : 512);
    if (S->pool) { const int nch = (nph + 63) / 64; return (nch < cap ? (nch > 0 ? nch : 1) : cap) + nlb + ndb; }
    const int total = nblk + nlb + ndb;
    return total < cap ? total : cap;
}

extern "C" int pc_update_fused_ok(const PcState *S, int nc) { return nc == 1 && S->D <= 128; }
extern "C" int pc_update_fused_blocks(const PcState *S, int nph)
{
    const int G = upd_grid(S, nph, 1), E = pc_update_fused_entries(S);
    return G + (G + UPD_FOLD - 1) / UPD_FOLD + (S->D * S->D + 2 + E - 1) / E;
}
extern "C" int pc_update_fused_entries(const PcState *S) { const int e = S->D * (S->D + 1) / 2 + S->D + 1; return (e + 31) & ~31; }

extern "C" void pc_launch_update_fused(const PcState *S, int nph, unsigned char *keep, int *blk, int *d_total, double *ph2, double *phL2,
                                       unsigned *phC2, unsigned long long *phU2, double *part, double *shift, int deferred, hipStream_t st)
{
    const int D = S->D, nblk = (nph + UPD_ROWS - 1) / UPD_ROWS, nlb = (S->Ncap + UPD_ROWS - 1) / UPD_ROWS, E = pc_update_fused_entries(S);
    const int ndb = deferred ? (S->B + UPD_ROWS - 1) / UPD_ROWS : 0;
    const int NTv = (D + 1 + 15) / 16, TSv = NTv <= 2 ? 16 * NTv + 1 : 16 * NTv + ((NTv & 1) ? 0 : 16), CAPv = NTv <= 2 ? 128 : 64;
    const int G = upd_grid(S, nph, deferred), ng = (G + UPD_FOLD - 1) / UPD_FOLD;
    double *part2 = part + (size_t)G * E;
    size_t shw = sizeof(double) * ((size_t)CAPv * TSv + D);
    if (NTv <= 2 && shw < sizeof(double) * (size_t)(4 * 3 * 256)) shw = sizeof(double) * (size_t)(4 * 3 * 256);
    hipLaunchKernelGGL(k_upd_flag, dim3((nblk + 3) / 4), dim3(UPD_NT), 0, st, *S, nph, keep, blk, deferred, nblk);
    if (!S->pool) pc_launch_scan_blocks(blk, nblk, d_total, &S->ctl->nphantom, st);
    else if (nblk <= UPD_SELF_BLOCKS && !std::getenv("PC_UPD_SCAN_LAUNCH"))
        hipLaunchKernelGGL(k_upd_index_self, dim3((nblk + 15) / 16), dim3(UPD_IDX_NT), 0, st, nph, (const unsigned char *)keep, (const int *)blk, nblk, (int *)phC2, d_total);
    else {
        hipLaunchKernelGGL(k_upd_scan, dim3(1), dim3(1024), 0, st, blk, nblk, d_total);
        hipLaunchKernelGGL(k_upd_index, dim3(nblk), dim3(UPD_NT), 0, st, nph, (const unsigned char *)keep, (const int *)blk, (int *)phC2);
    }
    int devi = 0; (void)hipGetDevice(&devi); devi &= 63;
#define UPDG_LAUNCH(NT) { \
        pc_need_dyn_lds((const void *)k_upd_gather<NT, false>, shw); \
                          pc_need_dyn_lds((const void *)k_upd_gather<NT, true>, shw); \
         \
        if (S->pool) hipLaunchKernelGGL((k_upd_gather<NT, true>), dim3(G), dim3(256), shw, st, *S, nph, nblk, (const unsigned char *)keep, (const int *)blk, \
                           ph2, phL2, phC2, phU2, (const int *)phC2, (const int *)d_total, (const double *)shift, part, E, deferred, nlb, ndb); \
        else hipLaunchKernelGGL((k_upd_gather<NT, false>), dim3(G), dim3(256), shw, st, *S, nph, nblk, (const unsigned char *)keep, (const int *)blk, \
                           ph2, phL2, phC2, phU2, (const int *)nullptr, (const int *)nullptr, (const double *)shift, part, E, deferred, nlb, ndb); }
    switch (NTv) { case 1: UPDG_LAUNCH(1) break; case 2: UPDG_LAUNCH(2) break; case 3: UPDG_LAUNCH(3) break; case 4: UPDG_LAUNCH(4) break;
                   case 5: UPDG_LAUNCH(5) break; case 6: UPDG_LAUNCH(6) break; case 7: UPDG_LAUNCH(7) break; case 8: UPDG_LAUNCH(8) break;
                   default: UPDG_LAUNCH(9) break; }
#undef UPDG_LAUNCH
    hipLaunchKernelGGL(k_upd_fold, dim3(ng), dim3(256), 0, st, (const double *)part, G, E, part2);
    if (D < 32) { hipLaunchKernelGGL(k_upd_final, dim3(1), dim3(1024), 0, st, *S, ng, (const double *)part2, E, shift, deferred); return; }
    double *ncov = part2 + (size_t)ng * E;
    int *count = (int *)(ncov + (size_t)D * D);
    const size_t shf = sizeof(double) * (size_t)(D * (D + 1) / 2 + D + 1);
    pc_need_dyn_lds((const void *)k_upd_final_w, shf);
    hipLaunchKernelGGL(k_upd_final_w, dim3(1), dim3(1024), shf, st, *S, ng, (const double *)part2, E, shift, deferred, ncov, count);
    pc_launch_chol_only(S, ncov, count, st);
}

extern "C" int pc_update_fused_grid(const PcState *S, int nph, int deferred) { return upd_grid(S, nph, deferred); }
extern "C" int pc_launch_update_fused_many(const PcState *S, const PcManyRec *dR, int R, int nblk_max, int G, int deferred, hipStream_t st)
{
    const int D = S->D, nlb = (S->Ncap + UPD_ROWS - 1) / UPD_ROWS, E = pc_update_fused_entries(S);
    if (!S->pool || nblk_max > UPD_SELF_BLOCKS || D >= 32 || nblk_max < 1) return 1;
    const int ndb = deferred ? (S->B + UPD_ROWS - 1) / UPD_ROWS : 0;
    const int NTv = (D + 1 + 15) / 16, TSv = NTv <= 2 ? 16 * NTv + 1 : 16 * NTv + ((NTv & 1) ? 0 : 16), CAPv = NTv <= 2 ? 128 : 64;
    const int ng = (G + UPD_FOLD - 1) / UPD_FOLD;
    size_t shw = sizeof(double) * ((size_t)CAPv * TSv + D);
    if (NTv <= 2 && shw < sizeof(double) * (size_t)(4 * 3 * 256)) shw = sizeof(double) * (size_t)(4 * 3 * 256);
    hipLaunchKernelGGL(k_upd_flag_many, dim3((nblk_max + 3) / 4, R), dim3(UPD_NT), 0, st, dR, deferred);
    hipLaunchKernelGGL(k_upd_index_self_many, dim3((nblk_max + 15) / 16, R), dim3(UPD_IDX_NT), 0, st, dR);
    int devi = 0; (void)hipGetDevice(&devi); devi &= 63;
#define UPDM_LAUNCH(NT) { \
        pc_need_dyn_lds((const void *)k_upd_gather_many<NT>, shw); \
        hipLaunchKernelGGL((k_upd_gather_many<NT>), dim3(G, R), dim3(256), shw, st, dR, E, deferred, nlb, ndb); }
    if (NTv == 1) UPDM_LAUNCH(1) else UPDM_LAUNCH(2)
#undef UPDM_LAUNCH
    hipLaunchKernelGGL(k_upd_fold_many, dim3(ng, R), dim3(256), 0, st, dR, G, E);
    hipLaunchKernelGGL(k_upd_final_many, dim3(1, R), dim3(1024), 0, st, dR, ng, E, deferred, G);
    return 0;
}
```

Before: 1.218 billion likelihood evals/s.

## Chain covariance update kernels with atomic tickets and shrink final kernel

Adds a fused flag+scan kernel and a chained gather kernel that use last-block atomic tickets, so the separate scan, index, fold and final launches of the covariance update can be merged into fewer launches. The gather path now builds index lists on the fly from block offsets, and dead-point staging uses compacted int indices with a shared staging helper. The final Cholesky kernel is templated on dimension bound and launched with 256 instead of 1024 threads. The new chained path only runs when an ablate bit (1<<16) is set, so by default only the reworked dead staging, the smaller final kernel and the write-through stores take effect.

```diff
diff --git a/polychordlite_amd/csrc/pc_engine.hip b/polychordlite_amd/csrc/pc_engine.hip
--- a/polychordlite_amd/csrc/pc_engine.hip
+++ b/polychordlite_amd/csrc/pc_engine.hip
@@ -847,7 +847,7 @@
         for (int r = 1; r < raw_depth; ++r) raw_buf[r] = ((D <= 24 || split_q || split_m) && S.nhat_raw) ? dalloc<double>(raw_n) : nullptr;
         S.plan = dalloc<PcPlan>(B); S.slot_src = dalloc<int>(Ncap); S.slot_step = dalloc<int>(Ncap); S.slot_dead = dalloc<int>(Ncap); HIPCHK(hipMemsetAsync(S.slot_dead, 0xFF, sizeof(int) * Ncap, st)); S.defer_update = 0; S.sort_slot = dalloc<int>(Ncap + 64); S.sort_key = dalloc<unsigned long long>(Ncap + 64);
         S.ctl = dalloc<PcCtl>(1);
-        d_total = dalloc<int>(1);
+        d_total = dalloc<int>(PC_UPD_CTR_INTS); HIPCHK(hipMemsetAsync(d_total, 0, sizeof(int) * PC_UPD_CTR_INTS, st));
         if (callback_mode) {
             d_cs = (void *)dalloc<char>(pc_chain_state_size() * B); d_x0s = dalloc<double>((size_t)B * D); d_prop = dalloc<double>((size_t)B * D);
             const size_t nans = (size_t)B * (1 + D + std::max(1, nDer));
diff --git a/polychordlite_amd/csrc/pc_launch.h b/polychordlite_amd/csrc/pc_launch.h
--- a/polychordlite_amd/csrc/pc_launch.h
+++ b/polychordlite_amd/csrc/pc_launch.h
@@ -91,6 +91,7 @@
 int pc_update_fused_ok(const PcState *S, int nc);
 int pc_update_fused_blocks(const PcState *S, int nph);
 int pc_update_fused_entries(const PcState *S);
+#define PC_UPD_CTR_INTS 2048
 void pc_launch_update_fused(const PcState *S, int nph, unsigned char *keep, int *blk, int *d_total, double *ph2, double *phL2, unsigned *phC2,
                             unsigned long long *phU2, double *part, double *shift, int deferred, hipStream_t st);
 int pc_update_fused_grid(const PcState *S, int nph, int deferred);
diff --git a/polychordlite_amd/csrc/pc_update.hip b/polychordlite_amd/csrc/pc_update.hip
--- a/polychordlite_amd/csrc/pc_update.hip
+++ b/polychordlite_amd/csrc/pc_update.hip
@@ -39,6 +39,7 @@
     }
 }
 
+template <typename T> __device__ __forceinline__ void upd_store_wt(T *p, T v) { __hip_atomic_store(p, v, __ATOMIC_RELAXED, __HIP_MEMORY_SCOPE_AGENT); }
 __device__ __forceinline__ void upd_flag_body(const PcState &S, int nph, unsigned char *keep, int *blk_count, int def, int nblk)
 {
     const int tid = threadIdx.x, lane = tid & 63, wv = tid >> 6;
@@ -81,10 +82,53 @@
     } else {
         for (int u = 0; u < 4; ++u) if (j0 + u < nph) { keep[j0 + u] = (unsigned char)((kb >> (8 * u)) & 0xFFu); if (wr) S.ph_cuid[j0 + u] = cu[u]; }
     }
-    if (lane == 0) blk_count[sb] = cnt;
+    if (lane == 0) upd_store_wt(blk_count + sb, cnt);
 }
 __global__ __launch_bounds__(UPD_NT) void k_upd_flag(PcState S, int nph, unsigned char *keep, int *blk_count, int def, int nblk) { upd_flag_body(S, nph, keep, blk_count, def, nblk); }
 __global__ __launch_bounds__(UPD_NT) void k_upd_flag_many(const PcManyRec *R, int def) { const PcManyView r = pc_many_view(R, blockIdx.y); if ((int)blockIdx.x * 4 >= r.ia[2]) return; upd_flag_body(r.S, r.ia[1], (unsigned char *)r.p[0], (int *)r.p[1], def, r.ia[2]); }
+
+__device__ __forceinline__ bool upd_ticket_last(int *ctr, int n, int *last_s)
+{
+    asm volatile("s_waitcnt vmcnt(0)" ::: "memory");
+    __syncthreads();
+    if (threadIdx.x == 0) {
+        const int t = __hip_atomic_fetch_add(ctr, 1, __ATOMIC_RELAXED, __HIP_MEMORY_SCOPE_AGENT);
+        const int last = t == n - 1;
+        if (last) {
+            __builtin_amdgcn_fence(__ATOMIC_ACQUIRE, "agent");
+            asm volatile("s_waitcnt vmcnt(0)" ::: "memory");
+            __hip_atomic_store(ctr, 0, __ATOMIC_RELAXED, __HIP_MEMORY_SCOPE_AGENT);
+        }
+        *last_s = last;
+    }
+    __syncthreads();
+    return *last_s != 0;
+}
+#define UPD_TICKET_FLAG 1
+#define UPD_TICKET_FINAL 2
+#define UPD_TICKET_GROUP 16
+
+#define UPD_SELF_BLOCKS 4096
+__global__ __launch_bounds__(UPD_NT) void k_upd_flag_scan(PcState S, int nph, unsigned char *keep, int *blk, int def, int nblk, int *ctr)
+{
+    __shared__ int last_s, wsum[4];
+    upd_flag_body(S, nph, keep, blk, def, nblk);
+    if (!upd_ticket_last(ctr + UPD_TICKET_FLAG, (int)gridDim.x, &last_s)) return;
+    const int tid = threadIdx.x, lane = tid & 63, wv = tid >> 6, i0 = 16 * tid;
+    int c[16], s = 0;
+#pragma unroll
+    for (int u = 0; u < 16; ++u) { c[u] = (i0 + u < nblk) ? blk[i0 + u] : 0; s += c[u]; }
+    int inc = s;
+#pragma unroll
+    for (int o = 1; o < 64; o <<= 1) { const int t = __shfl_up(inc, o); if (lane >= o) inc += t; }
+    if (lane == 63) wsum[wv] = inc;
+    __syncthreads();
+    int run = inc - s;
+    for (int x = 0; x < wv; ++x) run += wsum[x];
+#pragma unroll
+    for (int u = 0; u < 16; ++u) { if (i0 + u < nblk) blk[i0 + u] = run; run += c[u]; }
+    if (tid == UPD_NT - 1) ctr[0] = run;
+}
 
 
 __global__ __launch_bounds__(1024) void k_upd_scan(int *cnt, int n, int *total)
@@ -130,7 +174,6 @@
     if (km) idx[off + __popcll(m & ((1ull << lane) - 1ull))] = j;
 }
 
-#define UPD_SELF_BLOCKS 4096
 #define UPD_IDX_NT 256
 #define UPD_IDX_BLOCKS 16
 __device__ __forceinline__ void upd_index_self_body(int nph, const unsigned char *keep, const int *blk_count, int nblk, int *idx, int *total)
@@ -190,6 +233,120 @@
     }
 }
 
+#define UPD_FOLD 16
+__device__ __forceinline__ void upd_fold_body(const double *part, int nb, int E, double *part2, int g)
+{
+    for (int e = threadIdx.x; e < E; e += 256) {
+        double t[UPD_FOLD];
+#pragma unroll
+        for (int u = 0; u < UPD_FOLD; ++u) t[u] = (g * UPD_FOLD + u < nb) ? part[(size_t)(g * UPD_FOLD + u) * E + e] : 0.0;
+        double s = 0.0;
+#pragma unroll
+        for (int u = 0; u < UPD_FOLD; ++u) s += t[u];
+        upd_store_wt(part2 + (size_t)g * E + e, s);
+    }
+}
+__global__ __launch_bounds__(256) void k_upd_fold(const double *part, int nb, int E, double *part2) { upd_fold_body(part, nb, E, part2, blockIdx.x); }
+__global__ __launch_bounds__(256) void k_upd_fold_many(const PcManyRec *R, int nb, int E) { double *part = pc_as_global((double *)R[blockIdx.y].p[7], R); upd_fold_body(part, nb, E, part + (size_t)nb * E, blockIdx.x); }
+
+
+__device__ __forceinline__ void upd_final_fold(int nb, const double *part, int E, int nE, double *tot)
+{
+    for (int e = threadIdx.x; e < nE; e += 256) {
+        double s[4] = {0.0, 0.0, 0.0, 0.0};
+        for (int k0 = 0; k0 < nb; k0 += 4 * 16) {
+            double t[4][16];
+#pragma unroll
+            for (int h = 0; h < 4; ++h)
+#pragma unroll
+                for (int u = 0; u < 16; ++u) t[h][u] = (k0 + h + 4 * u < nb) ? part[(size_t)(k0 + h + 4 * u) * E + e] : 0.0;
+#pragma unroll
+            for (int h = 0; h < 4; ++h)
+#pragma unroll
+                for (int u = 0; u < 16; ++u) s[h] += t[h][u];
+        }
+        tot[e] = (s[0] + s[1]) + (s[2] + s[3]);
+    }
+    __syncthreads();
+}
+#define UPD_FINAL_LDS (544 + 1024 + 1024 + 32 + 1)
+template <int DMAX>
+__device__ __forceinline__ void upd_final_stage(const PcState &S, double *lds, double *shift, int def)
+{
+    double *tot = lds, *A = tot + 544, *L = A + 1024, *mu = L + 1024;
+    int *bad = (int *)(mu + 32);
+    const int tid = threadIdx.x, D = S.D, npair = D * (D + 1) / 2;
+#ifdef UPD_DBG
+    const long long f0 = clock64();
+#endif
+    if (tid == 0) *bad = 0;
+    const double n = tot[npair + D];
+    if (tid < D) mu[tid] = tot[npair + tid] / n;
+    __syncthreads();
+    for (int p = tid; p < D * D; p += 256) {
+        const int a = p / D, b = p % D, lo = a < b ? a : b, hi = a < b ? b : a;
+        const int idx = lo * D - lo * (lo - 1) / 2 + (hi - lo);
+        const double c = tot[idx] / n - mu[lo] * mu[hi];
+        A[p] = c; L[p] = 0.0;
+        S.cov[p] = c;
+    }
+    __syncthreads();
+#ifdef UPD_DBG
+    const long long f1 = clock64();
+#endif
+    if (tid < 64) {
+        double a[DMAX];
+#pragma unroll
+        for (int k = 0; k < DMAX; ++k) a[k] = (tid < D && k < D) ? A[tid * D + k] : 0.0;
+        bool fail = false;
+#pragma unroll
+        for (int i = 0; i < DMAX; ++i) {
+            if (i < D && !fail) {
+                const double aii = readlane_f64(a[i], i);
+                if (aii <= 0.0) fail = true;
+                else {
+                    const double lii = sqrt(aii);
+                    const double lji = (tid == i) ? lii : a[i] / lii;
+                    if (tid >= i) a[i] = lji;
+#pragma unroll
+                    for (int k = i + 1; k < DMAX; ++k) { const double lki = readlane_f64(lji, k); if (tid > i) a[k] -= lji * lki; }
+                }
+            }
+        }
+        if (fail) { if (tid == 0) *bad = 1; }
+        else if (tid < D) {
+#pragma unroll
+            for (int k = 0; k < DMAX; ++k) if (k < D) L[tid * D + k] = (k <= tid) ? a[k] : 0.0;
+        }
+    }
+    __syncthreads();
+    if (*bad) {
+        double tr = 0.0;
+        for (int k = 0; k < D; ++k) tr += A[k * D + k];
+        for (int p = tid; p < D * D; p += 256) L[p] = (p / D == p % D) ? sqrt(tr) : 0.0;
+        __syncthreads();
+    }
+    for (int p = tid; p < D * D; p += 256) S.chol[p] = L[p];
+    if (tid < D) shift[tid] += mu[tid];
+    if (tid == 0) { if (!(def && S.ctl->upd_keep_thr)) S.death_thr[0] = -PC_HUGE; if (def) S.ctl->upd_pending = 0; }
+#ifdef UPD_DBG
+    if (tid == 0) { const long long f2 = clock64(); S.ctl->gen_cyc[2] += f1 - f0; S.ctl->gen_cyc[3] += f2 - f1; S.ctl->nn_walks += f0; }
+#endif
+}
+template <int NT>
+__device__ __forceinline__ void upd_final_body(const PcState &S, int nb, const double *part, int E, double *lds, double *shift, int def)
+{
+    const int D = S.D;
+    upd_final_fold(nb, part, E, D * (D + 1) / 2 + D + 1, lds);
+    if (NT != 2 && D <= 8) upd_final_stage<8>(S, lds, shift, def);
+    else if (D <= 16) upd_final_stage<16>(S, lds, shift, def);
+    else if (NT != 1 && D <= 24) upd_final_stage<24>(S, lds, shift, def);
+    else if (NT != 1) upd_final_stage<32>(S, lds, shift, def);
+}
+__global__ __launch_bounds__(256) void k_upd_final(PcState S, int nb, const double *part, int E, double *shift, int def) { __shared__ double lds[UPD_FINAL_LDS]; upd_final_body<0>(S, nb, part, E, lds, shift, def); }
+__global__ __launch_bounds__(256) void k_upd_final_many(const PcManyRec *R, int nb, int E, int def, int G) { __shared__ double lds[UPD_FINAL_LDS]; const PcManyView r = pc_many_view(R, blockIdx.y); upd_final_body<0>(r.S, nb, (const double *)r.p[7] + (size_t)G * E, E, lds, (double *)r.p[8], def); }
+
+
 typedef double upd_v4d __attribute__((ext_vector_type(4)));
 template <int NT, int W>
 __device__ __forceinline__ void updg_accumulate(const double *tile, int TS, int n16, int wv, int li, int lk, upd_v4d (&acc)[(NT <= 2) ? NT * (NT + 1) / 2 : (NT * (NT + 1) / 2 + 3) / 4])
@@ -228,19 +385,20 @@
     return (b < D) ? a * D - a * (a - 1) / 2 + (b - a) : (a < D ? npair + a : npair + D);
 }
 
-template <int NT, bool IDX>
+template <int NT, bool IDX, bool CHAIN>
 __device__ __forceinline__ void upd_gather_body(const PcState &S, int nph, int nblk, const unsigned char *keep, const int *blk_off,
                                                 double *ph2, double *phL2, unsigned *phC2, unsigned long long *phU2,
                                                 const int *idx, const int *nidx_p,
-                                                const double *shift, double *part, int E, int def, int nlb, int ndb)
-{
+                                                const double *shift, double *part, int E, int def, int nlb, int ndb, double *shift_out = nullptr, int *ctr = nullptr)
+{
+    static_assert(!CHAIN || IDX, "the chain is pool mode's");
     extern __shared__ __attribute__((aligned(16))) char smem[];
     constexpr bool KS = NT <= 2;
     constexpr int TS = KS ? 16 * NT + 1 : 16 * NT + ((NT & 1) ? 0 : 16);
     constexpr int CAP = KS ? 128 : 64;
     constexpr int NACC = KS ? NT * (NT + 1) / 2 : (NT * (NT + 1) / 2 + 3) / 4;
     __shared__ unsigned long long m64[4], mm64[4];
-    __shared__ long long dix[256];
+    __shared__ int dix[256];
     const int tmark = def ? S.ctl->upd_tmark : 0x7fffffff, nph0u = def ? S.ctl->upd_nph0 : 0x7fffffff, updT = def ? S.ctl->upd_T : 0;
     const int tid = threadIdx.x, lane = tid & 63, wv = tid >> 6, li = lane & 15, lk = lane >> 4, D = S.D, nT = S.nT;
     constexpr bool pool = IDX;
@@ -252,6 +410,9 @@
 #pragma unroll
     for (int t = 0; t < NACC; ++t) acc[t] = upd_v4d{0.0, 0.0, 0.0, 0.0};
     int nfill = 0;
+#ifdef UPD_DBG
+    const long long g0 = clock64();
+#endif
     auto flush = [&]() __attribute__((always_inline)) {
         __syncthreads();
         const int n16 = (nfill + 15) & ~15;
@@ -276,6 +437,41 @@
     if constexpr (IDX) {
         const int nidx = *nidx_p;
         const int gchunk = (int)gridDim.x - nlb - ndb;
+        if constexpr (CHAIN) {
+            __shared__ int off_s[UPD_SELF_BLOCKS + 1], ridx_s[2][64];
+            const bool mine = (int)blockIdx.x < gchunk && (int)blockIdx.x * 64 < nidx;
+            if (mine) {
+                for (int b = tid; b < nblk; b += 256) off_s[b] = blk_off[b];
+                if (tid == 0) off_s[nblk] = nidx;
+                __syncthreads();
+            }
+            const unsigned long long below = (1ull << lane) - 1ull;
+            int par = 0;
+            for (int c = blockIdx.x; mine && c * 64 < nidx; c += gchunk, par ^= 1) {
+                const int p0 = c * 64, have = min(64, nidx - p0), p1 = p0 + have;
+                if (nfill + have > CAP) flush();
+                int lo = 0, hi = nblk - 1;
+                while (lo < hi) { const int mid = (lo + hi + 1) >> 1; if (off_s[mid] <= p0) lo = mid; else hi = mid - 1; }
+                for (int sb = lo + wv; sb < nblk; sb += 4) {
+                    const int o = off_s[sb];
+                    if (o >= p1) break;
+                    if (off_s[sb + 1] == o) continue;
+                    const int j0 = sb * UPD_ROWS + 4 * lane;
+                    unsigned w = 0;
+                    if (j0 + 3 < nph) w = *(const unsigned *)(keep + j0);
+                    else for (int u = 0; u < 4; ++u) if (j0 + u < nph) w |= (unsigned)keep[j0 + u] << (8 * u);
+                    int pos = o;
+                    bool f[4];
+#pragma unroll
+                    for (int u = 0; u < 4; ++u) { f[u] = (w >> (8 * u + 1)) & 1u; pos += __popcll(__ballot(f[u]) & below); }
+#pragma unroll
+                    for (int u = 0; u < 4; ++u) if (f[u]) { if (pos >= p0 && pos < p1) ridx_s[par][pos - p0] = j0 + u; pos++; }
+                }
+                __syncthreads();
+                upd_stage_idx(S.phantom, ridx_s[par] + 16 * wv, min(16, have - 16 * wv), tile + (size_t)(nfill + 16 * wv) * TS, TS, sh, D, nT, lane);
+                nfill += have;
+            }
+        } else
         for (int c = blockIdx.x; (int)blockIdx.x < gchunk && c * 64 < nidx; c += gchunk) {
             const int have = min(64, nidx - c * 64);
             if (nfill + have > CAP) flush();
@@ -320,35 +516,29 @@
             const PcCtl *ctl = S.ctl;
             const int T = ctl->upd_T, ts = ctl->upd_ts;
             const int t = tmark + (b - nblk - nlb) * 256 + tid;
-            long long di = -1;
+            int di = -1;
             if (t < ts) {
                 const PcPlan *pw = S.plan + (T - 1 - t);
                 const int src = pw->dead_src;
                 const bool existed = src >= 0 || (T - 1 - (-src - 1)) < tmark;
                 if (pw->dead_idx >= 0 && pw->logw > S.logzero && existed) di = pw->dead_idx;
             }
-            dix[tid] = di;
             const unsigned long long m = __ballot(di >= 0);
+            if (di >= 0) dix[wv * 64 + __popcll(m & ((1ull << lane) - 1ull))] = (int)di;
             if (lane == 0) m64[wv] = m;
             __syncthreads();
             for (int sub = 0; sub < 4; ++sub) {
-                unsigned long long mb = m64[sub];
-                const int cnt = __popcll(mb);
+                const int cnt = __popcll(m64[sub]);
                 if (cnt == 0) continue;
                 if (nfill + cnt > CAP) flush();
-                int row = 0;
-                while (mb) {
-                    const int bit = __ffsll((long long)mb) - 1; mb &= mb - 1;
-                    if ((row & 3) == wv) {
-                        const long long d = dix[sub * 64 + bit];
-                        for (int e = lane; e <= D; e += 64) tile[(size_t)(nfill + row) * TS + e] = e < D ? S.dead[(size_t)d * nT + e] - sh[e] : 1.0;
-                    }
-                    row++;
-                }
+                upd_stage_idx(S.dead, dix + sub * 64 + 16 * wv, min(16, cnt - 16 * wv), tile + (size_t)(nfill + 16 * wv) * TS, TS, sh, D, nT, lane);
                 nfill += cnt;
             }
         }
     }
+#ifdef UPD_DBG
+    const long long g1 = clock64();
+#endif
     flush();
     double *out = part + (size_t)blockIdx.x * E;
     if constexpr (KS) {
@@ -367,7 +557,7 @@
 #pragma unroll
                     for (int r = 0; r < 4; ++r) {
                         const int p = updg_slot(D, ti, tj, li, lk, r), idx = (lk + 4 * r) * 16 + li;
-                        if (p >= 0) out[p] = ((wres[(size_t)(0 * NACC + q) * 256 + idx] + wres[(size_t)(1 * NACC + q) * 256 + idx]) +
+                        if (p >= 0) upd_store_wt(out + p, (wres[(size_t)(0 * NACC + q) * 256 + idx] + wres[(size_t)(1 * NACC + q) * 256 + idx]) +
                                               (wres[(size_t)(2 * NACC + q) * 256 + idx] + wres[(size_t)(3 * NACC + q) * 256 + idx]));
                     }
         }
@@ -381,6 +571,23 @@
 #pragma unroll
                     for (int r = 0; r < 4; ++r) { const int p = updg_slot(D, ti, tj, li, lk, r); if (p >= 0) out[p] = acc[q >> 2][r]; }
                 }
+    }
+#ifdef UPD_DBG
+    if (IDX && tid == 0) {
+        const int gch = (int)gridDim.x - nlb - ndb, kind = (int)blockIdx.x < gch ? 0 : ((int)blockIdx.x < gch + nlb ? 1 : 2);
+        atomicAdd((unsigned long long *)&S.ctl->wave_cyc[kind], (unsigned long long)(g1 - g0));
+        atomicAdd((unsigned long long *)&S.ctl->wave_cyc[3], (unsigned long long)(clock64() - g1));
+    }
+#endif
+    if constexpr (CHAIN && KS) {
+        static_assert(sizeof(double) * UPD_FINAL_LDS <= sizeof(double) * 4 * 3 * 256, "the final stage's LDS fits the row tile");
+        __shared__ int last_s;
+        const int G = gridDim.x, g = blockIdx.x / UPD_FOLD, ng = (G + UPD_FOLD - 1) / UPD_FOLD;
+        double *part2 = part + (size_t)G * E;
+        if (!upd_ticket_last(ctr + UPD_TICKET_GROUP + g, min(UPD_FOLD, G - g * UPD_FOLD), &last_s)) return;
+        upd_fold_body(part, G, E, part2, g);
+        if (!upd_ticket_last(ctr + UPD_TICKET_FINAL, ng, &last_s)) return;
+        upd_final_body<NT>(S, ng, part2, E, tile, shift_out, def);
     }
 }
 template <int NT, bool IDX>
@@ -388,118 +595,17 @@
                                                     double *ph2, double *phL2, unsigned *phC2, unsigned long long *phU2,
                                                     const int *idx, const int *nidx_p,
                                                     const double *shift, double *part, int E, int def, int nlb, int ndb)
-{ upd_gather_body<NT, IDX>(S, nph, nblk, keep, blk_off, ph2, phL2, phC2, phU2, idx, nidx_p, shift, part, E, def, nlb, ndb); }
+{ upd_gather_body<NT, IDX, false>(S, nph, nblk, keep, blk_off, ph2, phL2, phC2, phU2, idx, nidx_p, shift, part, E, def, nlb, ndb); }
+template <int NT>
+__global__ __launch_bounds__(256) void k_upd_chain(PcState S, int nph, int nblk, const unsigned char *keep, const int *blk_off, double *shift, double *part, int E, int def, int nlb, int ndb, int *ctr)
+{ upd_gather_body<NT, true, true>(S, nph, nblk, keep, blk_off, nullptr, nullptr, nullptr, nullptr, nullptr, ctr, shift, part, E, def, nlb, ndb, shift, ctr); }
 template <int NT>
 __global__ __launch_bounds__(256) void k_upd_gather_many(const PcManyRec *R, int E, int def, int nlb, int ndb)
 {
     const PcManyView r = pc_many_view(R, blockIdx.y);
-    upd_gather_body<NT, true>(r.S, r.ia[1], r.ia[2], (const unsigned char *)r.p[0], (const int *)r.p[1], (double *)r.p[3], (double *)r.p[4], (unsigned *)r.p[5],
+    upd_gather_body<NT, true, false>(r.S, r.ia[1], r.ia[2], (const unsigned char *)r.p[0], (const int *)r.p[1], (double *)r.p[3], (double *)r.p[4], (unsigned *)r.p[5],
                               (unsigned long long *)r.p[6], (const int *)r.p[5], (const int *)r.p[2], (const double *)r.p[8], (double *)r.p[7], E, def, nlb, ndb);
 }
-
-
-#define UPD_FOLD 16
-__device__ __forceinline__ void upd_fold_body(const double *part, int nb, int E, double *part2)
-{
-    const int g = blockIdx.x;
-    for (int e = threadIdx.x; e < E; e += 256) {
-        double t[UPD_FOLD];
-#pragma unroll
-        for (int u = 0; u < UPD_FOLD; ++u) t[u] = (g * UPD_FOLD + u < nb) ? part[(size_t)(g * UPD_FOLD + u) * E + e] : 0.0;
-        double s = 0.0;
-#pragma unroll
-        for (int u = 0; u < UPD_FOLD; ++u) s += t[u];
-        part2[(size_t)g * E + e] = s;
-    }
-}
-__global__ __launch_bounds__(256) void k_upd_fold(const double *part, int nb, int E, double *part2) { upd_fold_body(part, nb, E, part2); }
-__global__ __launch_bounds__(256) void k_upd_fold_many(const PcManyRec *R, int nb, int E) { double *part = pc_as_global((double *)R[blockIdx.y].p[7], R); upd_fold_body(part, nb, E, part + (size_t)nb * E); }
-
-
-__device__ __forceinline__ void upd_final_body(const PcState &S, int nb, const double *part, int E, double *shift, int def)
-{
-    __shared__ double acc[4][256];
-    __shared__ double A[32 * 32], L[32 * 32], mu[32];
-    __shared__ int bad;
-    const int tid = threadIdx.x, D = S.D, npair = D * (D + 1) / 2, nE = npair + D + 1;
-    __shared__ double tot[544];
-    for (int e0 = 0; e0 < nE; e0 += 256) {
-        const int e = e0 + (tid & 255), h = tid >> 8;
-        double s = 0.0;
-        if (e < nE) {
-            for (int k = h; k < nb; k += 4 * 16) {
-                double t[16];
-#pragma unroll
-                for (int u = 0; u < 16; ++u) t[u] = (k + 4 * u < nb) ? part[(size_t)(k + 4 * u) * E + e] : 0.0;
-#pragma unroll
-                for (int u = 0; u < 16; ++u) s += t[u];
-            }
-        }
-        acc[h][tid & 255] = s;
-        __syncthreads();
-        if (tid < 256 && e < nE) tot[e] = (acc[0][tid] + acc[1][tid]) + (acc[2][tid] + acc[3][tid]);
-        __syncthreads();
-    }
-#ifdef UPD_DBG
-    const long long f0 = clock64();
-#endif
-    if (tid == 0) bad = 0;
-    const double n = tot[npair + D];
-    if (tid < D) mu[tid] = tot[npair + tid] / n;
-    __syncthreads();
-    for (int p = tid; p < D * D; p += 1024) {
-        const int a = p / D, b = p % D, lo = a < b ? a : b, hi = a < b ? b : a;
-        const int idx = lo * D - lo * (lo - 1) / 2 + (hi - lo);
-        const double c = tot[idx] / n - mu[lo] * mu[hi];
-        A[p] = c; L[p] = 0.0;
-        S.cov[p] = c;
-    }
-    __syncthreads();
-#ifdef UPD_DBG
-    const long long f1 = clock64();
-#endif
-    if (tid < 64) {
-        double a[32];
-#pragma unroll
-        for (int k = 0; k < 32; ++k) a[k] = (tid < D && k < D) ? A[tid * D + k] : 0.0;
-        bool fail = false;
-#pragma unroll
-        for (int i = 0; i < 32; ++i) {
-            if (i < D && !fail) {
-                const double aii = readlane_f64(a[i], i);
-                if (aii <= 0.0) fail = true;
-                else {
-                    const double lii = sqrt(aii);
-                    const double lji = (tid == i) ? lii : a[i] / lii;
-                    if (tid >= i) a[i] = lji;
-#pragma unroll
-                    for (int k = i + 1; k < 32; ++k)
-                        if (k < D) { const double lki = readlane_f64(lji, k); if (tid > i) a[k] -= lji * lki; }
-                }
-            }
-        }
-        if (fail) { if (tid == 0) bad = 1; }
-        else if (tid < D) {
-#pragma unroll
-            for (int k = 0; k < 32; ++k) if (k < D) L[tid * D + k] = (k <= tid) ? a[k] : 0.0;
-        }
-    }
-    __syncthreads();
-    if (bad) {
-        double tr = 0.0;
-        for (int k = 0; k < D; ++k) tr += A[k * D + k];
-        for (int p = tid; p < D * D; p += 1024) L[p] = (p / D == p % D) ? sqrt(tr) : 0.0;
-        __syncthreads();
-    }
-    for (int p = tid; p < D * D; p += 1024) S.chol[p] = L[p];
-    if (tid < D) shift[tid] += mu[tid];
-    if (tid == 0) { if (!(def && S.ctl->upd_keep_thr)) S.death_thr[0] = -PC_HUGE; if (def) S.ctl->upd_pending = 0; }
-#ifdef UPD_DBG
-    if (tid == 0) { const long long f2 = clock64(); S.ctl->gen_cyc[2] += f1 - f0; S.ctl->gen_cyc[3] += f2 - f1; S.ctl->nn_walks += f0; }
-#endif
-}
-__global__ __launch_bounds__(1024) void k_upd_final(PcState S, int nb, const double *part, int E, double *shift, int def) { upd_final_body(S, nb, part, E, shift, def); }
-__global__ __launch_bounds__(1024) void k_upd_final_many(const PcManyRec *R, int nb, int E, int def, int G) { const PcManyView r = pc_many_view(R, blockIdx.y); upd_final_body(r.S, nb, (const double *)r.p[7] + (size_t)G * E, E, (double *)r.p[8], def); }
 
 
 __global__ __launch_bounds__(1024) void k_upd_final_w(PcState S, int nb, const double *part, int E, double *shift, int def, double *ncov, int *count)
@@ -559,29 +665,42 @@
     double *part2 = part + (size_t)G * E;
     size_t shw = sizeof(double) * ((size_t)CAPv * TSv + D);
     if (NTv <= 2 && shw < sizeof(double) * (size_t)(4 * 3 * 256)) shw = sizeof(double) * (size_t)(4 * 3 * 256);
-    hipLaunchKernelGGL(k_upd_flag, dim3((nblk + 3) / 4), dim3(UPD_NT), 0, st, *S, nph, keep, blk, deferred, nblk);
-    if (!S->pool) pc_launch_scan_blocks(blk, nblk, d_total, &S->ctl->nphantom, st);
-    else if (nblk <= UPD_SELF_BLOCKS && !std::getenv("PC_UPD_SCAN_LAUNCH"))
-        hipLaunchKernelGGL(k_upd_index_self, dim3((nblk + 15) / 16), dim3(UPD_IDX_NT), 0, st, nph, (const unsigned char *)keep, (const int *)blk, nblk, (int *)phC2, d_total);
-    else {
-        hipLaunchKernelGGL(k_upd_scan, dim3(1), dim3(1024), 0, st, blk, nblk, d_total);
-        hipLaunchKernelGGL(k_upd_index, dim3(nblk), dim3(UPD_NT), 0, st, nph, (const unsigned char *)keep, (const int *)blk, (int *)phC2);
-    }
-    int devi = 0; (void)hipGetDevice(&devi); devi &= 63;
+    if (S->pool && nblk <= UPD_SELF_BLOCKS && UPD_TICKET_GROUP + ng <= PC_UPD_CTR_INTS && (S->ablate & (1 << 16))) {
+        int *ctr = d_total;
+        hipLaunchKernelGGL(k_upd_flag_scan, dim3((nblk + 3) / 4), dim3(UPD_NT), 0, st, *S, nph, keep, blk, deferred, nblk, ctr);
+#define UPDC_LAUNCH(NT) { \
+        pc_need_dyn_lds((const void *)k_upd_chain<NT>, shw); \
+        hipLaunchKernelGGL((k_upd_chain<NT>), dim3(G), dim3(256), shw, st, *S, nph, nblk, (const unsigned char *)keep, (const int *)blk, shift, part, E, deferred, nlb, ndb, ctr); }
+        switch (NTv) { case 1: UPDC_LAUNCH(1) break; case 2: UPDC_LAUNCH(2) break; case 3: UPDC_LAUNCH(3) break; case 4: UPDC_LAUNCH(4) break;
+                       case 5: UPDC_LAUNCH(5) break; case 6: UPDC_LAUNCH(6) break; case 7: UPDC_LAUNCH(7) break; case 8: UPDC_LAUNCH(8) break;
+                       default: UPDC_LAUNCH(9) break; }
+#undef UPDC_LAUNCH
+        if (D < 32) return;
+    } else {
+        hipLaunchKernelGGL(k_upd_flag, dim3((nblk + 3) / 4), dim3(UPD_NT), 0, st, *S, nph, keep, blk, deferred, nblk);
+        if (!S->pool) pc_launch_scan_blocks(blk, nblk, d_total, &S->ctl->nphantom, st);
+        else if (nblk <= UPD_SELF_BLOCKS && !std::getenv("PC_UPD_SCAN_LAUNCH"))
+            hipLaunchKernelGGL(k_upd_index_self, dim3((nblk + 15) / 16), dim3(UPD_IDX_NT), 0, st, nph, (const unsigned char *)keep, (const int *)blk, nblk, (int *)phC2, d_total);
+        else {
+            hipLaunchKernelGGL(k_upd_scan, dim3(1), dim3(1024), 0, st, blk, nblk, d_total);
+            hipLaunchKernelGGL(k_upd_index, dim3(nblk), dim3(UPD_NT), 0, st, nph, (const unsigned char *)keep, (const int *)blk, (int *)phC2);
+        }
+        int devi = 0; (void)hipGetDevice(&devi); devi &= 63;
 #define UPDG_LAUNCH(NT) { \
-        pc_need_dyn_lds((const void *)k_upd_gather<NT, false>, shw); \
-                          pc_need_dyn_lds((const void *)k_upd_gather<NT, true>, shw); \
-         \
-        if (S->pool) hipLaunchKernelGGL((k_upd_gather<NT, true>), dim3(G), dim3(256), shw, st, *S, nph, nblk, (const unsigned char *)keep, (const int *)blk, \
-                           ph2, phL2, phC2, phU2, (const int *)phC2, (const int *)d_total, (const double *)shift, part, E, deferred, nlb, ndb); \
-        else hipLaunchKernelGGL((k_upd_gather<NT, false>), dim3(G), dim3(256), shw, st, *S, nph, nblk, (const unsigned char *)keep, (const int *)blk, \
-                           ph2, phL2, phC2, phU2, (const int *)nullptr, (const int *)nullptr, (const double *)shift, part, E, deferred, nlb, ndb); }
-    switch (NTv) { case 1: UPDG_LAUNCH(1) break; case 2: UPDG_LAUNCH(2) break; case 3: UPDG_LAUNCH(3) break; case 4: UPDG_LAUNCH(4) break;
-                   case 5: UPDG_LAUNCH(5) break; case 6: UPDG_LAUNCH(6) break; case 7: UPDG_LAUNCH(7) break; case 8: UPDG_LAUNCH(8) break;
-                   default: UPDG_LAUNCH(9) break; }
+            pc_need_dyn_lds((const void *)k_upd_gather<NT, false>, shw); \
+                              pc_need_dyn_lds((const void *)k_upd_gather<NT, true>, shw); \
+             \
+            if (S->pool) hipLaunchKernelGGL((k_upd_gather<NT, true>), dim3(G), dim3(256), shw, st, *S, nph, nblk, (const unsigned char *)keep, (const int *)blk, \
+                               ph2, phL2, phC2, phU2, (const int *)phC2, (const int *)d_total, (const double *)shift, part, E, deferred, nlb, ndb); \
+            else hipLaunchKernelGGL((k_upd_gather<NT, false>), dim3(G), dim3(256), shw, st, *S, nph, nblk, (const unsigned char *)keep, (const int *)blk, \
+                               ph2, phL2, phC2, phU2, (const int *)nullptr, (const int *)nullptr, (const double *)shift, part, E, deferred, nlb, ndb); }
+        switch (NTv) { case 1: UPDG_LAUNCH(1) break; case 2: UPDG_LAUNCH(2) break; case 3: UPDG_LAUNCH(3) break; case 4: UPDG_LAUNCH(4) break;
+                       case 5: UPDG_LAUNCH(5) break; case 6: UPDG_LAUNCH(6) break; case 7: UPDG_LAUNCH(7) break; case 8: UPDG_LAUNCH(8) break;
+                       default: UPDG_LAUNCH(9) break; }
 #undef UPDG_LAUNCH
+    }
     hipLaunchKernelGGL(k_upd_fold, dim3(ng), dim3(256), 0, st, (const double *)part, G, E, part2);
-    if (D < 32) { hipLaunchKernelGGL(k_upd_final, dim3(1), dim3(1024), 0, st, *S, ng, (const double *)part2, E, shift, deferred); return; }
+    if (D < 32) { hipLaunchKernelGGL(k_upd_final, dim3(1), dim3(256), 0, st, *S, ng, (const double *)part2, E, shift, deferred); return; }
     double *ncov = part2 + (size_t)ng * E;
     int *count = (int *)(ncov + (size_t)D * D);
     const size_t shf = sizeof(double) * (size_t)(D * (D + 1) / 2 + D + 1);
@@ -609,6 +728,6 @@
     if (NTv == 1) UPDM_LAUNCH(1) else UPDM_LAUNCH(2)
 #undef UPDM_LAUNCH
     hipLaunchKernelGGL(k_upd_fold_many, dim3(ng, R), dim3(256), 0, st, dR, G, E);
-    hipLaunchKernelGGL(k_upd_final_many, dim3(1, R), dim3(1024), 0, st, dR, ng, E, deferred, G);
+    hipLaunchKernelGGL(k_upd_final_many, dim3(1, R), dim3(256), 0, st, dR, ng, E, deferred, G);
     return 0;
 }
```

After: 1.277 billion likelihood evals/s (median of 6 runs). +4.9%, better.
